# COPT-Public/LoRADS

Hardware: AMD Instinct MI355X
Metric: ADMM iters/sec (+ inner CG-iters/sec), single-block n=20000 r=40 (higher is better)
Workload: dtype f64

## Files before the change

### include/lorads_hip.h

```cpp
#ifndef LORADS_HIP_H
#define LORADS_HIP_H

#include <stdint.h>

#ifdef __cplusplus
extern "C" {
#endif

typedef struct lorads_hip_ctx lorads_hip_ctx;

typedef struct {
    int32_t n;
    int32_t rank;
    int32_t nrow;
    const int32_t *row_idx;
    const int32_t *a_ptr;
    const int32_t *a_row;
    const int32_t *a_col;
    const double *a_val;
    int32_t c_nnz;
    const int32_t *c_row;
    const int32_t *c_col;
    const double *c_val;
    int32_t is_lp;
// ... 19 lines not shown
void lorads_hip_destroy(lorads_hip_ctx *ctx);
const char *lorads_hip_last_error(void);

int lorads_hip_init_constr(lorads_hip_ctx *ctx, int32_t pair);
int lorads_hip_alm_cal_grad(lorads_hip_ctx *ctx, double rho, double *lag_norm_sq);
int lorads_hip_lbfgs_direction(lorads_hip_ctx *ctx, int32_t inner_iter);
int lorads_hip_alm_q12p12(lorads_hip_ctx *ctx, double p12[2]);
int lorads_hip_alm_linesearch_coeffs(lorads_hip_ctx *ctx, double rho, double p1, double p2, double coef[4]);
int lorads_hip_set_y_as_neg_grad(lorads_hip_ctx *ctx);
int lorads_hip_alm_update_var(lorads_hip_ctx *ctx, double tau);
int lorads_hip_set_lbfgs_his_two(lorads_hip_ctx *ctx, double tau);
int lorads_hip_update_dimacs(lorads_hip_ctx *ctx, int32_t pair, double *err1);
int lorads_hip_cal_obj(lorads_hip_ctx *ctx, int32_t pair, double *pobj);
int lorads_hip_alm_front(lorads_hip_ctx *ctx, double rho, int32_t inner, double out[6]);
int lorads_hip_alm_step(lorads_hip_ctx *ctx, double rho, double tau, int32_t next_inner, double out[8]);
int lorads_hip_admm_update_var(lorads_hip_ctx *ctx, double rho, double cg_tol, int32_t cg_max_iter,
                               int32_t *cg_iters);
int lorads_hip_admm_step(lorads_hip_ctx *ctx, double rho, double cg_tol, int32_t cg_max_iter, double out[4]);
int lorads_hip_update_dual_var(lorads_hip_ctx *ctx, double rho);
int lorads_hip_cal_dual_obj(lorads_hip_ctx *ctx, double *dobj);

int lorads_hip_dual_infeasibility(lorads_hip_ctx *ctx, double tol, int32_t ncv, int32_t max_restarts, double *sum_neg,
                                  double *lam_min, int32_t *matvecs);

#define LORADS_HIP_CERT_N 10
int lorads_hip_certificate(lorads_hip_ctx *ctx, int32_t src, double tol, int32_t ncv, int32_t max_restarts,
                           double out[LORADS_HIP_CERT_N], double *lam_min, double *residual, double *lambda);
int lorads_hip_get_slack(lorads_hip_ctx *ctx, int32_t blk, int64_t *nnz, int32_t *row, int32_t *col, double *val);

int lorads_hip_round_pm1(lorads_hip_ctx *ctx, int32_t src, int32_t trials, uint64_t seed, int32_t max_rounds, double *obj,
                         double *obj0, int32_t *best, int32_t *best0, int8_t *sign, int32_t *rounds, double *hyperplanes);

int lorads_hip_round_kcut(lorads_hip_ctx *ctx, int32_t src, int32_t parts, int32_t trials, uint64_t seed, int32_t max_rounds,
                          double *obj, double *obj0, int32_t *best, int32_t *best0, uint8_t *label, int32_t *rounds, double *vectors,
                          double *t, double *lp_upper);

int lorads_hip_round_stable(lorads_hip_ctx *ctx, int32_t src, int32_t trials, uint64_t seed, int32_t max_rounds, double *obj,
                            double *obj0, int32_t *best, int32_t *best0, uint8_t *member, int32_t *sizes, int32_t *rounds,
                            double *scores, double *T);

int lorads_hip_round_bisect(lorads_hip_ctx *ctx, int32_t src, int32_t trials, uint64_t seed, int32_t max_rounds, double *obj,
                            double *obj0, int32_t *best, int32_t *best0, int8_t *sign, int32_t *imbalance, int32_t *rounds,
                            double *hyperplanes, double *t, int32_t *diff);

int lorads_hip_spectrum(lorads_hip_ctx *ctx, int32_t src, double *eig, double *q, int32_t *sweeps);
int lorads_hip_compress_rank(lorads_hip_ctx *ctx, int32_t src, const int32_t *new_rank, double *eig);

#define LORADS_HIP_PRIMAL_CHUNK 262144
#define LORADS_HIP_PRIMAL_EPW 128
int lorads_hip_primal_entries(lorads_hip_ctx *ctx, int32_t src, int32_t blk, int64_t count, const int32_t *row, const int32_t *col,
                              double *val, const double *ref, double stats[4]);
int lorads_hip_primal_apply(lorads_hip_ctx *ctx, int32_t src, int32_t blk, int32_t ncols, const double *B, double *Y, double *T);

int lorads_hip_triangle_cuts(lorads_hip_ctx *ctx, int32_t src, int32_t blk, double min_violation, int32_t max_cuts, int64_t *count,
                             int32_t *p, int32_t *q, int32_t *s, int8_t *cls, double *viol, int32_t *kept, int32_t *passes);

int lorads_hip_entry_bounds(lorads_hip_ctx *ctx, int32_t src, int32_t blk, double lower, double upper, double min_violation,
                            int32_t max_cuts, int64_t *count, int32_t *p, int32_t *q, int8_t *cls, double *viol, int32_t *kept,
                            int32_t *passes);

int lorads_hip_primal_topk(lorads_hip_ctx *ctx, int32_t src, int32_t blk, int32_t nq, const int32_t *row, int32_t col_lo, int32_t col_hi,
                           int32_t k, int32_t smallest, int32_t include_diag, const int64_t *skip_ptr, const int32_t *skip_col,
                           int32_t *idx, double *val, int32_t *found);

int lorads_hip_alm_to_admm(lorads_hip_ctx *ctx);
int lorads_hip_average_uv_to_v(lorads_hip_ctx *ctx);
int lorads_hip_scale_obj(lorads_hip_ctx *ctx, double s);
int lorads_hip_resize_rank(lorads_hip_ctx *ctx, const int32_t *new_rank);
int lorads_hip_set_mat(lorads_hip_ctx *ctx, int32_t which, int32_t blk, const double *colmajor);
int lorads_hip_get_mat(lorads_hip_ctx *ctx, int32_t which, int32_t blk, double *colmajor);
int lorads_hip_set_vec(lorads_hip_ctx *ctx, int32_t which, const double *v);
int lorads_hip_get_vec(lorads_hip_ctx *ctx, int32_t which, double *v);
int lorads_hip_set_allreduce(lorads_hip_ctx *ctx, lorads_hip_allreduce_fn fn, void *user);
void *lorads_hip_stream(lorads_hip_ctx *ctx);
int lorads_hip_set_allreduce_stream_ordered(lorads_hip_ctx *ctx, int32_t on);
int lorads_hip_set_separable(lorads_hip_ctx *ctx, int32_t on);
typedef int (*lorads_hip_scalar_exchange_fn)(void *user, double *vals, int32_t n);
int lorads_hip_set_scalar_exchange(lorads_hip_ctx *ctx, lorads_hip_scalar_exchange_fn fn, void *user);
int lorads_hip_selfcheck_allreduce(lorads_hip_ctx *ctx);

int lorads_hip_sync(lorads_hip_ctx *ctx);
int lorads_hip_spec_front_stats(lorads_hip_ctx *ctx, int64_t out[4]);
int lorads_hip_handover_stats(lorads_hip_ctx *ctx, int64_t out[2]);
int lorads_hip_row_deal_stats(lorads_hip_ctx *ctx, int32_t block, int out[3]);
int lorads_hip_wt_stores(lorads_hip_ctx *ctx, int *mask);
int lorads_hip_front_chain(lorads_hip_ctx *ctx, int *mask, int *effective);
int lorads_hip_dense_plan(lorads_hip_ctx *ctx, int32_t block, int64_t out[16]);

#ifdef __cplusplus
}
#endif
#endif
```

### lorads_amd/csrc/hip/build.inc

```
struct HostPattern {
    std::vector<int> erow, ecol;
    std::vector<int> e_ptr, e_con;
    std::vector<double> e_val;
    std::vector<int> adj_ptr, adj_col, adj_e;
};
#include "presolve.inc"

void unique_positions(const std::vector<std::pair<int, int>> &pos, std::vector<std::pair<int, int>> &uniq,
                      std::vector<int> &index) {
    std::vector<int> order(pos.size());
    for (size_t i = 0; i < pos.size(); ++i) order[i] = (int)i;
    std::sort(order.begin(), order.end(), [&](int a, int b) {
        if (pos[a].second != pos[b].second) return pos[a].second < pos[b].second;
        if (pos[a].first != pos[b].first) return pos[a].first < pos[b].first;
        return a < b;
    });
    uniq.clear();
    index.assign(pos.size(), -1);
    for (size_t k = 0; k < order.size(); ++k) {
        int i = order[k];
        if (uniq.empty() || uniq.back() != pos[i]) uniq.push_back(pos[i]);
        index[i] = (int)uniq.size() - 1;
    }
}
// ... 333 lines not shown
    }
    tm.lap("operator kind (diag / single entry / colouring)");
    if (!diag && !B.dense_a && build_gram(M, B, hb, a_e, B.pa.ne)) return 1;
    tm.lap("Gram");
    {
        int maxsz = 0;
        for (int i = 0; i < hb.nrow; ++i) maxsz = std::max(maxsz, hb.a_ptr[i + 1] - hb.a_ptr[i]);
        const char *force = getenv("LORADS_OP_CW");
        bool want = !diag && !B.entry_only && hb.nrow >= 256 && maxsz <= 512;
        if (force && !diag && !B.entry_only && hb.nrow > 0) want = force[0] == '1';
        if (B.dense_a) want = false;
        if (want) {
            std::vector<int> deg(B.n + 1, 0);
            for (int t = 0; t < B.na; ++t) {
                deg[hb.a_row[t] + 1]++;
                if (hb.a_row[t] != hb.a_col[t]) deg[hb.a_col[t] + 1]++;
            }
            std::vector<int> ptr(B.n + 1, 0);
            for (int i = 0; i < B.n; ++i) ptr[i + 1] = ptr[i] + deg[i + 1];
            std::vector<int> col(ptr[B.n]), con(ptr[B.n]), fill(ptr.begin(), ptr.end() - 1);
            std::vector<double> av(ptr[B.n]);
            for (int i = 0; i < hb.nrow; ++i)
                for (int t = hb.a_ptr[i]; t < hb.a_ptr[i + 1]; ++t) {
                    const int p = hb.a_row[t], q = hb.a_col[t];
                    col[fill[p]] = q; con[fill[p]] = i; av[fill[p]] = hb.a_val[t]; fill[p]++;
                    if (p != q) { col[fill[q]] = p; con[fill[q]] = i; av[fill[q]] = hb.a_val[t]; fill[q]++; }
                }
            for (int i = 0; i < B.n; ++i) {
                const int s0 = ptr[i], s1 = ptr[i + 1];
                std::vector<std::tuple<int, int, double>> tmp(s1 - s0);
                for (int k = s0; k < s1; ++k) tmp[k - s0] = std::make_tuple(col[k], con[k], av[k]);
                std::sort(tmp.begin(), tmp.end());
                for (int k = s0; k < s1; ++k) { col[k] = std::get<0>(tmp[k - s0]); con[k] = std::get<1>(tmp[k - s0]); av[k] = std::get<2>(tmp[k - s0]); }
            }
            std::vector<int> car(hb.a_row, hb.a_row + B.na), cac(hb.a_col, hb.a_col + B.na);
            std::vector<double> cav(hb.a_val, hb.a_val + B.na);
            if (maxsz <= 32 && (double)hb.nrow * maxsz <= 1.5 * (double)B.na && !getenv("LORADS_NO_ELL")) {
                B.ca_ell = maxsz;
                car.assign((size_t)hb.nrow * maxsz, 0); cac.assign((size_t)hb.nrow * maxsz, 0); cav.assign((size_t)hb.nrow * maxsz, 0.0);
                for (int i = 0; i < hb.nrow; ++i)
                    for (int t = hb.a_ptr[i]; t < hb.a_ptr[i + 1]; ++t) {
                        const size_t w = (size_t)i * maxsz + (size_t)(t - hb.a_ptr[i]);
                        car[w] = hb.a_row[t]; cac[w] = hb.a_col[t]; cav[w] = hb.a_val[t];
                    }
            }
            if (!getenv("LORADS_NO_SLOT_ELL")) {
                long over8 = 0;
                for (int i = 0; i < B.n; ++i) over8 += (ptr[i + 1] - ptr[i]) > 8;
                const int ew = (double)over8 <= 0.005 * (double)B.n ? 8 : 16;
                std::vector<int> ecol((size_t)B.n * ew), econ((size_t)B.n * ew, 0);
                std::vector<double> eav((size_t)B.n * ew, 0.0);
                for (int i = 0; i < B.n; ++i)
                    for (int s = 0; s < ew; ++s) {
                        const int k = ptr[i] + s;
                        const size_t w = (size_t)i * ew + s;
                        if (k < ptr[i + 1]) { ecol[w] = col[k]; econ[w] = con[k]; eav[w] = av[k]; }
                        else ecol[w] = i;
                    }
                if (M.upload(&B.cell_col, ecol) || M.upload(&B.cell_con, econ) || M.upload(&B.cell_a, eav)) return 1;
                B.cell_w = ew;
            }
            if (B.cell_w && !B.dense_c && !getenv("LORADS_NO_FRONT_CW_DATA")) {
                std::vector<std::pair<int, int>> posC(B.nc), uniqC;
                for (int t = 0; t < B.nc; ++t) posC[t] = {hb.c_row[t], hb.c_col[t]};
                std::vector<int> cidx;
                unique_positions(posC, uniqC, cidx);
                std::vector<double> cval(uniqC.size(), 0.0);
                for (int t = 0; t < B.nc; ++t) cval[cidx[t]] += hb.c_val[t];
                HostPattern hpC;
                build_adjacency(B.n, uniqC, hpC);
                std::vector<double> fval(hpC.adj_e.size());
                for (size_t k = 0; k < hpC.adj_e.size(); ++k) fval[k] = cval[hpC.adj_e[k]];
                std::vector<int> ccount(hb.nrow, 0);
                for (int k = 0; k < ptr[B.n]; ++k) ccount[con[k]]++;
                int csw = 1;
                for (int i = 0; i < hb.nrow; ++i) csw = std::max(csw, ccount[i]);
                if ((double)hb.nrow * csw > 4.0 * (double)ptr[B.n] + 1024.0) csw = 0;
                if (csw > 0) {
                    std::vector<int> dstc(ptr[B.n]), fillc(hb.nrow, 0), dste((size_t)B.n * B.cell_w, 0);
                    for (int k = 0; k < ptr[B.n]; ++k) dstc[k] = con[k] * csw + fillc[con[k]]++;
                    for (int i = 0; i < B.n; ++i)
                        for (int sl = 0; sl < B.cell_w && ptr[i] + sl < ptr[i + 1]; ++sl) dste[(size_t)i * B.cell_w + sl] = dstc[ptr[i] + sl];
                    if (M.upload(&B.fc_ptr, hpC.adj_ptr) || M.upload(&B.fc_col, hpC.adj_col) || M.upload(&B.fc_val, fval) ||
                        M.upload(&B.cadj_dst, dstc) || M.upload(&B.cell_dst, dste) || M.alloc(&B.w_contrib, (size_t)hb.nrow * csw))
                        return 1;
                    HC(hipMemset(B.w_contrib, 0, sizeof(double) * std::max<size_t>((size_t)hb.nrow * csw, 1)));
                    B.cs_w = csw;
                    B.fc_nslot = (int)fval.size();
                    B.front_cw = true;
                }
            }
            if (M.upload(&B.ca_row, car) || M.upload(&B.ca_col, cac) || M.upload(&B.ca_val, cav) ||
                M.upload(&B.cadj_ptr, ptr) || M.upload(&B.cadj_col, col) || M.upload(&B.cadj_con, con) || M.upload(&B.cadj_a, av) ||
                M.alloc(&B.w_uv, (size_t)B.nrow) || M.alloc(&B.w_op, (size_t)B.nrow) || M.alloc(&B.pu.S2, (size_t)2 * B.pu.ne))
                return 1;
            B.cadj_ptr_host_n = ptr[B.n];
            B.use_cw = true;
        }
    }
    tm.lap("constraint-wise operator lists");
    if (hb.is_lp) {
        for (int t = 0; t < B.na; ++t)
            if (hb.a_row[t] != hb.a_col[t]) return fail_msg("LP block: off-diagonal entry");
        for (int t = 0; t < B.nc; ++t)
            if (hb.c_row[t] != hb.c_col[t]) return fail_msg("LP block: off-diagonal objective entry");
        const int n = B.n;
        std::vector<int> ptr(n + 1, 0), grow(B.na), fill(n, 0);
        std::vector<double> av(B.na), nrm(n, 0.0), cobj(n, 0.0);
        for (int t = 0; t < B.na; ++t) ptr[hb.a_row[t] + 1]++;
        for (int j = 0; j < n; ++j) ptr[j + 1] += ptr[j];
        for (int i = 0; i < hb.nrow; ++i)
            for (int t = hb.a_ptr[i]; t < hb.a_ptr[i + 1]; ++t) {
                const int col = hb.a_row[t], w = ptr[col] + fill[col]++;
                grow[w] = hb.row_idx[i];
                av[w] = hb.a_val[t];
            }
        for (int j = 0; j < n; ++j) {
            double nn = 0.0;
            for (int t = ptr[j]; t < ptr[j + 1]; ++t) nn += av[t] * av[t];
            const double nr = std::sqrt(nn);
            nrm[j] = nr * nr;
        }
        for (int t = 0; t < B.nc; ++t) cobj[hb.c_row[t]] += hb.c_val[t];
        std::vector<int> row_lvl((size_t)std::max(c->m, 1), 0), lvl(n, 0);
        int nlev = 0;
        for (int j = 0; j < n; ++j) {
            int l = 0;
            for (int t = ptr[j]; t < ptr[j + 1]; ++t) l = std::max(l, row_lvl[grow[t]]);
            lvl[j] = l;
            for (int t = ptr[j]; t < ptr[j + 1]; ++t) row_lvl[grow[t]] = l + 1;
            nlev = std::max(nlev, l + 1);
        }
        std::vector<int> lptr(nlev + 1, 0), lcols(n);
        for (int j = 0; j < n; ++j) lptr[lvl[j] + 1]++;
        for (int l = 0; l < nlev; ++l) lptr[l + 1] += lptr[l];
        std::vector<int> lf(lptr.begin(), lptr.end() - 1);
        for (int j = 0; j < n; ++j) lcols[lf[lvl[j]]++] = j;
        if (M.upload(&B.lp_ptr, ptr) || M.upload(&B.lp_grow, grow) || M.upload(&B.lp_a, av) || M.upload(&B.lp_nrm2sq, nrm) ||
            M.upload(&B.lp_cobj, cobj) || M.upload(&B.lp_lvl_ptr, lptr) || M.upload(&B.lp_lvl_cols, lcols) ||
            M.alloc(&B.lp_cv, (size_t)B.na))
            return 1;
        HC(hipMemset(B.lp_cv, 0, sizeof(double) * (size_t)std::max(B.na, 1)));
        B.is_lp = true;
        B.lp_nlev = nlev;
    }
    return 0;
}

void block_bytes(Block &B) {
    double F = 8.0 * B.n * B.r;
    B.bytes_mv = 4 * F + 32.0 * B.na + 16.0 * B.nrow;
    B.bytes_cg = B.bytes_mv + 9 * F;
}

inline int pad_rows(int n) { return (n + 31) & ~31; }

void common_rank(lorads_hip_ctx *c) {
    if (!c->merged_ok || c->nb < 2 || !env_on("LORADS_COMMON_RANK")) return;
    int rmax = 0;
    for (auto &B : c->blk) rmax = std::max(rmax, B.r);
    for (auto &B : c->blk) B.r = rmax;
}

int alloc_factors(lorads_hip_ctx *c) {
    c->all_elem = 0;
    for (auto &B : c->blk) {
        B.off = c->all_elem;
// ... 164 lines not shown
```

### lorads_amd/csrc/hip/dev.inc

```
int lorads_hip_ubench(lorads_hip_ctx *c, int32_t which, int32_t reps, double *ms) {
    spec_touch(c);
    if (c->nb < 1) return fail_msg("ubench: no cone");
    Block &B = c->blk[0];
    if (which >= 100) {
        if (!B.entry_only) return fail_msg("ubench: variants >= 100 need a single-entry cone");
        hipEvent_t e0, e1;
        HC(hipEventCreate(&e0)); HC(hipEventCreate(&e1));
        if (which != 100 && which != 120 && which != 121) return fail_msg("ubench: unknown variant");
        const Shape shp = shape_for(B.r);
        for (int it = -3; it < reps; ++it) {
            if (it == 0) HC(hipEventRecord(e0, c->stream));
            if (which == 100)
                op_entry(c, B, c->V + B.off, OP_CG, c->U + B.off, nullptr, c->cQ + B.off, part_slot(c, 0), NOGUARD);
            else
                SHAPE_DISPATCH(shp, LAUNCH((k_gather_probe<LG_, V2_, NS_>), nblocks_for((size_t)B.n, TPB / shp.lg), B.n, 16, B.pa.adj_col,
                                           B.na, c->V + B.off, which == 121 ? c->U + B.off : (const double *)nullptr, B.r,
                                           c->cQ + B.off));
        }
        HC(hipEventRecord(e1, c->stream));
        HC(hipEventSynchronize(e1));
        float f = 0;
        HC(hipEventElapsedTime(&f, e0, e1));
        *ms = f;
        hipEventDestroy(e0); hipEventDestroy(e1);
        return 0;
    }
    if (B.r != 40 || !B.use_cw || !B.cell_w || !B.pu.S2) return fail_msg("ubench: needs a k_cw cone of rank 40");
    const double *U = c->U + B.off, *V = c->V + B.off;
    double *Q = c->cQ + B.off, *r = c->cr + B.off, *p = c->cp + B.off, *rhs = c->rhs + B.off;
    const size_t len = (size_t)B.n * B.r;
    hipLaunchKernelGGL(k_fill, dim3(64), dim3(TPB), 0, c->stream, (size_t)NSLOT * c->maxpart, 1.0, c->part);
    HC(hipMemsetAsync(c->st, 0, sizeof(CGState) * 2, c->stream));
    hipEvent_t e0, e1;
    HC(hipEventCreate(&e0)); HC(hipEventCreate(&e1));
    const int grow = nblocks_for((size_t)B.n, TPB / 8), gcw = nblocks_for((size_t)B.nrow, TPB / 64);
    const RowDeal rd = row_deal_of(c, B);
    for (int it = -3; it < reps; ++it) {
        if (it == 0) HC(hipEventRecord(e0, c->stream));
        switch (which) {
        case 0: LAUNCH((k_cw<8, true, 3>), gcw, B.nrow, B.a_ptr, B.ca_row, B.ca_val, B.ca_col, U, V, B.r, 1.0, B.w_op, (double *)nullptr,
                       (int)CV_SET, B.row_idx, (double *)nullptr, NOGUARD, B.ca_ell, InitArgs{}, ResArgs{}); break;
        case 1: LAUNCH((k_cw<4, true, 5, true>), gcw, B.nrow, B.a_ptr, B.ca_row, B.ca_val, B.ca_col, U, V, B.r, 1.0, B.w_op,
                       (double *)nullptr, (int)CV_SET, B.row_idx, (double *)nullptr, NOGUARD, B.ca_ell, InitArgs{}, ResArgs{}); break;
        case 2:
            if (B.cell_w == 8) LAUNCH((k_spmm_ell<8, true, 3, 8>), rd.grid, B.n, rd.rpw, B.cadj_ptr, B.cadj_col, B.cadj_con, B.cadj_a, B.cell_col,
                                      B.cell_con, B.cell_a, (const double *)B.w_op, V, B.r, (int)OP_CG, U, (const double *)nullptr, Q,
                                      part_slot(c, 0), NOGUARD);
            else LAUNCH((k_spmm_ell<8, true, 3, 16>), rd.grid, B.n, rd.rpw, B.cadj_ptr, B.cadj_col, B.cadj_con, B.cadj_a, B.cell_col, B.cell_con,
                        B.cell_a, (const double *)B.w_op, V, B.r, (int)OP_CG, U, (const double *)nullptr, Q, part_slot(c, 0), NOGUARD);
            break;
        case 30: case 31: case 33: case 34: {
            if (!B.front_cw) return fail_msg("ubench: cone without the one-kernel front's data");
            FrontCwArgs A{};
            A.fc_ptr = B.fc_ptr; A.fc_col = B.fc_col; A.fc_val = B.fc_val; A.sl_ptr = B.cadj_ptr; A.sl_col = B.cadj_col; A.sl_con = B.cadj_con;
            A.sl_a = B.cadj_a; A.ell_col = B.cell_col; A.ell_con = B.cell_con; A.ell_a = B.cell_a; A.ell_dst = B.cell_dst; A.sl_dst = B.cadj_dst;
            A.csum = c->csum; A.b = c->b; A.lambda = c->lambda; A.cv = B.cv; A.w_uv = B.w_op;
            A.row_idx = B.row_idx_identity ? nullptr : B.row_idx; A.rho = 1.0; A.wmode = W_ADMM;
            A.contrib = (which == 30 || which == 33) ? B.w_contrib : (double *)nullptr;
            A.wt = c->opt_wt_stores;
            const size_t lds = sizeof(double2) * 32 * 4 * 3 * 8;
#define UB_FRONT(EWV, FCV) LAUNCH_LDS((k_front_cw<3, EWV, 4, false, FCV>), rd.grid, lds, B.n, rd.rpw, A, V, B.r, U, r, rhs, part_slot(c, 0), part_slot(c, 1), NOGUARD, Deferred{})
            if (which < 33) { if (B.cell_w == 8) UB_FRONT(8, 0); else UB_FRONT(16, 0); }
            else { if (B.cell_w == 8) UB_FRONT(8, FC_ALL); else UB_FRONT(16, FC_ALL); }
#undef UB_FRONT
        } break;
        case 32: LAUNCH(k_wsum, nblocks_for((size_t)B.nrow, TPB / 8), B.nrow, B.cs_w, (const double *)B.w_contrib, B.w_op, NOGUARD, InitArgs{}, 0, DS(0.0),
                        c->m, (const double *)c->b, (const double *)c->csum, c->lambda); break;
        case 3: LAUNCH((k_spmm<8, true, 3, true>), grow, B.n, B.cadj_ptr, B.cadj_col, B.cadj_con, (const double *)B.w_op, V, B.r,
                       (int)OP_CG, U, (const double *)nullptr, 0.0, Q, part_slot(c, 0), NOGUARD, (const double *)nullptr, B.cadj_a); break;
        case 4: LAUNCH((k_spmm2<8, true, 3, true>), grow, B.n, B.pu.adj_ptr, B.pu.adj_col, B.pu.adj_dyn, B.pu.adj_sval, B.pu.S, (const double *)B.pu.S2, V,
                       B.r, 0, U, (const double *)nullptr, 1.0, r, rhs, part_slot(c, 0), part_slot(c, 1), NOGUARD,
                       (const double *)nullptr); break;
        case 5: LAUNCH((k_spmm2<8, true, 3, false>), grow, B.n, B.pu.adj_ptr, B.pu.adj_col, B.pu.adj_dyn, B.pu.adj_sval, B.pu.S, (const double *)nullptr, V,
                       B.r, (int)OP_RHS, (const double *)nullptr, (const double *)nullptr, 1.0, rhs, (double *)nullptr, part_slot(c, 1),
                       (double *)nullptr, NOGUARD, (const double *)nullptr); break;
        case 6: case 7: case 8: case 9: {
            const int gv = 2048 >> (which - 6);
            LAUNCH(k_cg_update<true>, gv, len, c->st, part_slot(c, 0), 625, Q, rhs, p, r, part_slot(c, 2), NOGUARD, (double *)nullptr,
                   (const double *)nullptr, 0, c->st_shadow);
        } break;
        case 20: case 21: case 22: case 23: case 24: {
            const bool shortk = which >= 23;
            const int ngroups = shortk ? B.n : 40000, per = shortk ? 16 : 64;
            const double *two = (which == 21 || which == 24) ? U : (const double *)nullptr;
            const int *idx = which == 22 ? (const int *)nullptr : B.cadj_col;
            const int nidx = which == 22 ? B.n : B.cadj_ptr_host_n;
            if (nidx <= 0) return fail_msg("ubench: empty index list");
            LAUNCH((k_gather_probe<8, true, 3>), nblocks_for((size_t)ngroups, TPB / 8), ngroups, per, idx, nidx, V, two, B.r, Q);
        } break;
        case 25: LAUNCH((k_gather_probe2<8, true, 3, 0>), grow, B.n, B.pu.adj_ptr, B.pu.adj_col, B.pu.adj_e, B.pu.S, V, B.r, Q); break;
        case 26: LAUNCH((k_gather_probe2<8, true, 3, 1>), grow, B.n, B.pu.adj_ptr, B.pu.adj_col, B.pu.adj_e, B.pu.S, V, B.r, Q); break;
        case 27: LAUNCH((k_gather_probe2<8, true, 3, 3>), grow, B.n, B.pu.adj_ptr, B.pu.adj_col, B.pu.adj_e, B.pu.S, V, B.r, Q); break;
        case 28: LAUNCH((k_gather_probe2<8, true, 3, 7>), grow, B.n, B.pu.adj_ptr, B.pu.adj_col, B.pu.adj_e, B.pu.S, V, B.r, Q); break;
        case 10: case 13: case 14:
            LAUNCH((k_obj<8, true, 3>), std::min(nblocks_for((size_t)B.nc, TPB / 8), which == 10 ? 1024 : which == 13 ? 2048 : 4096), B.nc,
                   B.c_row, B.c_col, B.c_val, U, U, B.r, part_slot(c, 4), NOGUARD); break;
        case 11: LAUNCH(k_sval, std::max(1, nblocks_for((size_t)B.pu.ne, TPB)), B.pu.ne, B.pu.e_ptr, B.pu.e_con, B.pu.e_val, B.pu.cbase,
                        (int)W_COMPACT, WArgs{B.w_op, nullptr, nullptr, nullptr, nullptr, nullptr, 1.0}, B.pu.S, NOGUARD,
                        (CGState *)nullptr, 0, (const double *)B.w_op, B.pu.S2); break;
        default: return fail_msg("ubench: unknown variant");
        }
    }
    HC(hipEventRecord(e1, c->stream));
    HC(hipEventSynchronize(e1));
    float f = 0;
    HC(hipEventElapsedTime(&f, e0, e1));
    *ms = f;
    hipEventDestroy(e0); hipEventDestroy(e1);
    invalidate_t(c);
    return 0;
}
```

### lorads_amd/csrc/hip/kernels.inc

```
template <int LG, bool V2, int NS>
struct Slice {
    static constexpr int W = V2 ? 2 : 1;
    __device__ static __forceinline__ void load(const double *__restrict__ row, int r, int lane, double (&v)[NS][W]) {
#pragma unroll
        for (int c = 0; c < NS; ++c) {
            const int j = (lane + c * LG) * W;
            const bool ok = j < r;
            const int jc = ok ? j : 0;
            if (V2) {
                const double2 t = *(const double2 *)(row + jc);
                v[c][0] = ok ? t.x : 0.0;
                v[c][W - 1] = ok ? t.y : 0.0;
            } else {
                const double t = row[jc];
                v[c][0] = ok ? t : 0.0;
            }
        }
    }
    __device__ static __forceinline__ void load_raw(const double *__restrict__ row, int r, int lane, double (&v)[NS][W]) {
        static_assert(V2, "the 16-byte form only");
#pragma unroll
        for (int c = 0; c < NS; ++c) {
            const int j = (lane + c * LG) * W;
            const double2 t = *(const double2 *)(row + (j < r ? j : 0));
// ... 62 lines not shown
    double *part_v, *part_d;
};
template <int LG, bool V2, int NS, bool ONE = false>
__global__ __launch_bounds__(TPB) void k_cw(int nrow, const int *__restrict__ a_ptr, const int *__restrict__ a_p,
                                            const double *__restrict__ a_val, const int *__restrict__ a_q,
                                            const double *__restrict__ X,
                                            const double *__restrict__ Y, int r, double scale, double *__restrict__ w_out,
                                            double *__restrict__ cv, int mode, const int *__restrict__ row_idx,
                                            double *__restrict__ vec, Guard g, int ell_w, InitArgs ia, ResArgs ra,
                                            Deferred d = Deferred{}) {
    __shared__ double sh[8];
    DefPriv dv{};
    if (d.st) dv = deferred_private(d);
    const Gate gt = gate_load(ia.st ? Guard{nullptr, g.need} : g);
    double iv[2] = {0.0, 0.0};
    const bool ia_small = ia.st && ia.nrr <= 4 * TPB && ia.nb <= 4 * TPB;
    double ipr[2][4] = {{0.0, 0.0, 0.0, 0.0}, {0.0, 0.0, 0.0, 0.0}};
    if (ia_small) {
#pragma unroll
        for (int k = 0; k < 4; ++k) {
            const int j = threadIdx.x + k * TPB;
            ipr[0][k] = ia.part_rr[j < ia.nrr ? j : 0];
            ipr[1][k] = ia.part_b[j < ia.nb ? j : 0];
        }
    } else if (ia.st) init_private(ia, iv);
    constexpr int GR = 64 / LG;
    const int i = (blockIdx.x * TPB + threadIdx.x) >> 6, lane64 = threadIdx.x & 63;
    const int grp = lane64 / LG, lane = lane64 % LG;
    const bool act = i < nrow;
    const int ic = act ? i : 0;
    int gi_pre = 0;
    double b_pre = 0.0, l_pre = 0.0;
    if (ra.b) { gi_pre = row_idx[ic]; b_pre = ra.b[gi_pre]; l_pre = ra.lambda[gi_pre]; }
    const int t0 = ell_w ? ic * ell_w : a_ptr[ic], t1 = !act ? t0 : ell_w ? t0 + ell_w : a_ptr[ic + 1];
    double acc = 0.0;
    if (ONE) {
        for (int t = t0 + grp; t < t1; t += GR) {
            const int p0 = a_p[t], q0 = a_q[t];
            const double c0 = a_val[t];
            acc += c0 * pair_dot<LG, V2, NS>(X, Y, p0, q0, r, lane);
        }
    } else
    for (int t = t0 + grp; t < t1; t += 2 * GR) {
        const int tb = t + GR < t1 ? t + GR : t;
        const int p0 = a_p[t], q0 = a_q[t], p1 = a_p[tb], q1 = a_q[tb];
        const double c0 = a_val[t], c1 = t + GR < t1 ? a_val[tb] : 0.0;
        const double d0 = pair_dot<LG, V2, NS>(X, Y, p0, q0, r, lane);
        const double d1 = pair_dot<LG, V2, NS>(X, Y, p1, q1, r, lane);
        acc += c0 * d0;
        acc += c1 * d1;
    }
    const double s = wave_sum(acc);
    if (ia_small) {
#pragma unroll
        for (int k = 0; k < 4; ++k) {
            const int j = threadIdx.x + k * TPB;
            iv[0] += j < ia.nrr ? ipr[0][k] : 0.0;
            iv[1] += j < ia.nb ? ipr[1][k] : 0.0;
        }
    }
    const bool live = ia.st ? finish_init(ia, !(g.need && gt.vn == 0), iv, sh) == 0
                            : d.st ? !blocked_after(g, d, finish_deferred(d, dv, sh).done) : GATE_OPEN;
    if (live && act && lane64 == 0) {
        if (w_out) w_out[i] = s;
        if (vec) {
            const int gi = ra.b ? gi_pre : row_idx[i];
            if (mode == CV_SET) vec[gi] = s * scale;
            else if (mode == CV_ADD) vec[gi] += s * scale;
            else vec[gi] += s - cv[i];
        }
        if (cv) cv[i] = s;
    }
    if (ra.b) {
        double vd[2] = {0.0, 0.0};
        if (act && lane64 == 0) {
            const double bi = b_pre, t = bi - s * scale;
            vd[0] = t * t;
            vd[1] = bi * l_pre;
        }
        block_sum_n<2>(vd, sh);
        if (live && threadIdx.x == 0) { ra.part_v[blockIdx.x] = vd[0]; ra.part_d[blockIdx.x] = vd[1]; }
    }
}

template <int NS4, int NS>
__global__ __launch_bounds__(TPB) void k_eval_cw_obj(int nrow, int ell_w, const int *__restrict__ a_p, const double *__restrict__ a_val,
                                                     const int *__restrict__ a_q, const double *__restrict__ R, int r,
                                                     double *__restrict__ cv, const int *__restrict__ row_idx, double *__restrict__ vec,
                                                     ResArgs ra, int g_cw, int ne, const int *__restrict__ erow,
                                                     const int *__restrict__ ecol, const double *__restrict__ cval,
                                                     double *__restrict__ part_obj, Guard g, Deferred d) {
    __shared__ double sh[8];
    const Gate gt = gate_load(g);
    DefPriv dv{};
    if (d.st) dv = deferred_private(d);
    if ((int)blockIdx.x < g_cw) {
        constexpr int LG = 4, GR = 16;
        const int i = (blockIdx.x * TPB + threadIdx.x) >> 6, lane64 = threadIdx.x & 63;
        const int grp = lane64 / LG, lane = lane64 % LG;
        const bool act = i < nrow;
        const int ic = act ? i : 0;
        const int gi = row_idx[ic];
        const double bi = ra.b[gi], li = ra.lambda[gi];
        const int t0 = ic * ell_w, t1 = act ? t0 + ell_w : t0;
        double acc = 0.0;
        for (int t = t0 + grp; t < t1; t += GR) {
            const int p0 = a_p[t], q0 = a_q[t];
            const double c0 = a_val[t];
            acc += c0 * pair_dot<LG, true, NS4>(R, R, p0, q0, r, lane);
        }
        const double s = wave_sum(acc);
        const bool live = d.st ? !blocked_after(g, d, finish_deferred(d, dv, sh).done) : GATE_OPEN;
        if (live && act && lane64 == 0) { vec[gi] = s * 1.0; cv[i] = s; }
        double vd[2] = {0.0, 0.0};
        if (act && lane64 == 0) {
            const double t = bi - s * 1.0;
            vd[0] = t * t;
            vd[1] = bi * li;
        }
        block_sum_n<2>(vd, sh);
        if (live && threadIdx.x == 0) { ra.part_v[blockIdx.x] = vd[0]; ra.part_d[blockIdx.x] = vd[1]; }
        return;
    }
    constexpr int LG = 8, per = TPB / LG;
    const int bid = blockIdx.x - g_cw, nblk = gridDim.x - g_cw;
    const int lane = threadIdx.x % LG;
    double sacc = 0.0;
    for (int e = bid * per + threadIdx.x / LG; e < ne; e += nblk * per)
        sacc += pair_dot<LG, true, NS>(R, R, erow[e], ecol[e], r, lane) * cval[e];
    const bool live = d.st ? !blocked_after(g, d, finish_deferred(d, dv, sh).done) : GATE_OPEN;
    const double t = block_sum(sacc, sh);
    if (live && threadIdx.x == 0) part_obj[bid] = t;
}

__global__ void k_fill(size_t len, double v, double *__restrict__ y) {
    for (size_t i = (size_t)blockIdx.x * blockDim.x + threadIdx.x; i < len; i += (size_t)gridDim.x * blockDim.x) y[i] = v;
}

template <int LG, bool V2, int NS>
__device__ __forceinline__ void pair_dot_rd(const double *__restrict__ R, const double *__restrict__ D, int p, int q, int r,
                                            int lane, double &t1, double &t2) {
    constexpr int W = V2 ? 2 : 1;
    double rp[NS][W], rq[NS][W], dp[NS][W], dq[NS][W];
    Slice<LG, V2, NS>::load(R + (size_t)p * r, r, lane, rp);
    Slice<LG, V2, NS>::load(D + (size_t)q * r, r, lane, dq);
    Slice<LG, V2, NS>::load(R + (size_t)q * r, r, lane, rq);
    Slice<LG, V2, NS>::load(D + (size_t)p * r, r, lane, dp);
    double a1 = 0.0, a2 = 0.0, b1 = 0.0, b2 = 0.0;
#pragma unroll
    for (int c = 0; c < NS; ++c)
#pragma unroll
        for (int w = 0; w < W; ++w) {
            a1 += rp[c][w] * dq[c][w]; a2 += rq[c][w] * dp[c][w];
            b1 += dp[c][w] * dq[c][w]; b2 += dq[c][w] * dp[c][w];
        }
    t1 = p == q ? a1 : a1 + a2;
    t2 = p == q ? b1 : b1 + b2;
}
template <int LG, bool V2, int NS>
__global__ __launch_bounds__(TPB) void k_pairdots_rd(int ne, const int *__restrict__ erow, const int *__restrict__ ecol,
                                                     const double *__restrict__ R, const double *__restrict__ D, int r,
                                                     double *__restrict__ T1, double *__restrict__ T2) {
    const int e = (blockIdx.x * TPB + threadIdx.x) / LG, lane = threadIdx.x % LG;
    const bool act = e < ne;
    const int p = act ? erow[e] : 0, q = act ? ecol[e] : 0;
    double t1, t2;
// ... 356 lines not shown
                for (int u = 0; u < CH; ++u) {
                    const double a1 = __shfl(s1, u0 + u, 8);
                    const double a2 = FRONT ? __shfl(s2, u0 + u, 8) : 0.0;
#pragma unroll
                    for (int c = 0; c < NS; ++c)
#pragma unroll
                        for (int w = 0; w < W; ++w) {
                            acc[c][w] += a1 * v[u][c][w];
                            if (FRONT) acc2[c][w] += a2 * v[u][c][w];
                        }
                }
            }
        }
    }
    const bool live_ = (FRONT && d.st) ? !blocked_after(g, d, finish_deferred(d, dv, sh).done) : GATE_OPEN;
    double dd = 0.0;
    if (FRONT && gd) {
#pragma unroll
        for (int c = 0; c < NS; ++c)
#pragma unroll
            for (int w = 0; w < W; ++w) dd += rh[c][w] * xi[c][w];
        dd = group_sum<LG>(dd);
        if (uv_out && act && lane == 0 && live_) uv_out[rowc] = dd;
        dd *= gd[rowc];
    }
    double local = 0.0, local_b = 0.0;
#pragma unroll
    for (int c = 0; c < NS; ++c) {
        const int j0 = (lane + c * LG) * W;
        double v[W], vb[W];
#pragma unroll
        for (int w = 0; w < W; ++w) {
            const double a = acc[c][w];
            if (FRONT) {
                vb[w] = xi[c][w] - a / rho; local_b += fabs(vb[w]);
                const double opx = gd ? rh[c][w] + dd * xi[c][w] : rh[c][w] + acc2[c][w];
                v[w] = vb[w] - opx; local += v[w] * v[w];
            } else if (mode == OP_CG) { v[w] = xi[c][w] + a; local += xi[c][w] * v[w]; }
            else if (mode == OP_RES) { v[w] = rh[c][w] - (xi[c][w] + a); local += v[w] * v[w]; }
            else if (mode == OP_RHS) { v[w] = xi[c][w] - a / rho; local += fabs(v[w]); }
            else { v[w] = 2.0 * a; local += v[w] * v[w]; }
        }
        if (live_ && act && j0 < r) {
            if (V2) *(double2 *)(out + base + j0) = make_double2(v[0], v[W - 1]);
            else out[base + j0] = v[0];
            if (FRONT) {
                if (V2) *(double2 *)(rhs_out + base + j0) = make_double2(vb[0], vb[W - 1]);
                else rhs_out[base + j0] = vb[0];
            }
        }
    }
    if (FRONT) {
        double two[2] = {act ? local : 0.0, act ? local_b : 0.0};
        block_sum_n<2>(two, sh);
        if (live_ && threadIdx.x == 0) { part[blockIdx.x] = two[0]; part_b[blockIdx.x] = two[1]; }
    } else {
        const double t = block_sum(act ? local : 0.0, sh);
        if (live_ && threadIdx.x == 0) part[blockIdx.x] = t;
    }
}

struct Cg0Args {
    const CGState *st;
    const double *part_ww;
    int nww;
    double *x, *r;
    int store_r;
    double *w_acc;
    const double *w_p;
    int nw;
    CGState *shadow;
    const double *avg_other;
    double *avg_out;
    int wt;
};
struct CgElem { double x, r; };
__device__ __forceinline__ CgElem cg_elem(double alpha, double p, double q, double x, double r) {
    return CgElem{x + alpha * p, r - alpha * q};
}
__device__ __forceinline__ double cg_avg(double other, double x) { return (other + x) / 2; }
__device__ __forceinline__ double cg_wacc(double wa, double alpha, double wp) { return wa + alpha * wp; }
__device__ __forceinline__ double cg0_alpha(double rr, double ww) { return rr / (rr + ww); }

template <int LG, bool V2, int NS, int EW, bool CG0 = false>
__global__ __launch_bounds__(TPB) void k_spmm_ell(int n, int rpw, const int *__restrict__ adj_ptr, const int *__restrict__ adj_col,
                                                  const int *__restrict__ adj_con, const double *__restrict__ adj_a,
                                                  const int *__restrict__ ell_col, const int *__restrict__ ell_con,
                                                  const double *__restrict__ ell_a, const double *__restrict__ wgt,
                                                  const double *__restrict__ X, int r, int mode,
                                                  const double *xin, const double *__restrict__ rhs,
                                                  double *__restrict__ out, double *__restrict__ part, Guard g,
                                                  Cg0Args u = Cg0Args{}) {
    __shared__ double sh[4];
    const Gate gt = gate_load(g);
    double rr = 0.0, ww = 0.0, wa0 = 0.0, wp0 = 0.0;
    const int gid = blockIdx.x * TPB + threadIdx.x;
    if (CG0) {
        rr = u.st->rr;
        ww = private_partials(u.part_ww, u.nww);
        if (u.w_acc) { const int iw = gid < u.nw ? gid : 0; wa0 = u.w_acc[iw]; wp0 = u.w_p[iw]; }
    }
    constexpr int W = V2 ? 2 : 1;
    constexpr int NH = EW / 8;
    constexpr int CH = NS <= 5 ? 4 : 2;
    const int grp = threadIdx.x / LG, row = blockIdx.x * rpw + grp, lane = threadIdx.x % LG;
    const bool act = grp < rpw && row < n;
    const int rowc = act ? row : 0;
    const size_t base = (size_t)rowc * r;
    const size_t eb = (size_t)rowc * EW + (lane & 7);
    int qc[NH], kc[NH];
    double ac[NH];
#pragma unroll
    for (int h = 0; h < NH; ++h) { qc[h] = ell_col[eb + 8 * h]; kc[h] = ell_con[eb + 8 * h]; ac[h] = ell_a[eb + 8 * h]; }
    const int t0 = adj_ptr[rowc], t1r = adj_ptr[rowc + 1];
    const int t1 = act ? t1r : t0;
    double xi[NS][W], rh[NS][W], acc[NS][W];
    Slice<LG, V2, NS>::load(xin + base, r, lane, xi);
    Slice<LG, V2, NS>::load((CG0 ? (const double *)u.x : mode == OP_RES ? rhs : xin) + base, r, lane, rh);
#pragma unroll
    for (int c = 0; c < NS; ++c)
#pragma unroll
        for (int w = 0; w < W; ++w) acc[c][w] = 0.0;
    double wv[NH];
#pragma unroll
    for (int h = 0; h < NH; ++h) wv[h] = wgt[kc[h]];
    const int cnt = act ? t1 - t0 : 0;
#pragma unroll
    for (int h = 0; h < NH; ++h) {
        if (h == 0 || cnt > 8 * h) {
#pragma unroll
            for (int u0 = 0; u0 < 8; u0 += CH) {
                if (u0 > 0 && cnt <= 8 * h + u0) continue;
                double v[CH][NS][W];
#pragma unroll
                for (int u = 0; u < CH; ++u) {
                    const int q = __shfl(qc[h], u0 + u, 8);
                    Slice<LG, V2, NS>::load(X + (size_t)q * r, r, lane, v[u]);
                }
                const double sch = (lane & 7) + 8 * h < cnt ? ac[h] * wv[h] : 0.0;
#pragma unroll
                for (int u = 0; u < CH; ++u) {
                    const double su = __shfl(sch, u0 + u, 8);
#pragma unroll
                    for (int c = 0; c < NS; ++c)
#pragma unroll
                        for (int w = 0; w < W; ++w) acc[c][w] += su * v[u][c][w];
                }
            }
        }
    }
    constexpr int TU = CG0 ? 2 : 4;
    for (int t = t0 + EW; t < t1; t += TU) {
        int q[TU], e[TU];
        double aa[TU];
#pragma unroll
        for (int u = 0; u < TU; ++u) {
            const int tt = t + u < t1 ? t + u : t1 - 1;
            q[u] = adj_col[tt];
            e[u] = adj_con[tt];
            aa[u] = adj_a[tt];
        }
        double s4[TU], v[TU][NS][W];
#pragma unroll
        for (int u = 0; u < TU; ++u) {
            s4[u] = aa[u] * wgt[e[u]];
            Slice<LG, V2, NS>::load(X + (size_t)q[u] * r, r, lane, v[u]);
        }
#pragma unroll
        for (int u = 0; u < TU; ++u) {
            const double su = t + u < t1 ? s4[u] : 0.0;
#pragma unroll
            for (int c = 0; c < NS; ++c)
#pragma unroll
                for (int w = 0; w < W; ++w) acc[c][w] += su * v[u][c][w];
        }
    }
    if (CG0) {
        const double alpha = cg0_alpha(rr, block_sum(ww, sh));
        const bool open = GATE_OPEN;
        const bool avg_only = !open && gt.vs != 0 && !(g.need && gt.vn == 0);
        if (open && blockIdx.x == 0 && threadIdx.x == 0 && u.shadow) *u.shadow = *u.st;
        if (open && u.w_acc && gid < u.nw) {
            u.w_acc[gid] = cg_wacc(wa0, alpha, wp0);
            for (int i = gid + gridDim.x * TPB; i < u.nw; i += gridDim.x * TPB) u.w_acc[i] = cg_wacc(u.w_acc[i], alpha, u.w_p[i]);
        }
        double local = 0.0;
#pragma unroll
        for (int c = 0; c < NS; ++c) {
            const int j0 = (lane + c * LG) * W;
            double xo[W], ro[W];
#pragma unroll
            for (int w = 0; w < W; ++w) {
                const CgElem e = cg_elem(alpha, xi[c][w], xi[c][w] + acc[c][w], rh[c][w], xi[c][w]);
                xo[w] = e.x; ro[w] = e.r;
                local += e.r * e.r;
            }
            if (act && j0 < r) {
                if (open) {
                    if (V2) store16(u.x, base + j0, xo[0], xo[W - 1], u.wt & WT_CG0);
                    else store8(u.x, base + j0, xo[0], u.wt & WT_CG0);
                    if (u.store_r) {
                        if (V2) store16(u.r, base + j0, ro[0], ro[W - 1], u.wt & WT_CG0);
                        else store8(u.r, base + j0, ro[0], u.wt & WT_CG0);
                    }
                }
                if (u.avg_out && (open || avg_only)) {
                    double ao[W];
#pragma unroll
                    for (int w = 0; w < W; ++w) ao[w] = open ? xo[w] : rh[c][w];
                    if (V2) {
                        const double2 o = *(const double2 *)(u.avg_other + base + j0);
                        store16(u.avg_out, base + j0, cg_avg(o.x, ao[0]), cg_avg(o.y, ao[W - 1]), u.wt & WT_AVG);
                    } else {
                        store8(u.avg_out, base + j0, cg_avg(u.avg_other[base + j0], ao[0]), u.wt & WT_AVG);
                    }
                }
            }
        }
        const double t = block_sum(act ? local : 0.0, sh);
        if (open && threadIdx.x == 0) part[blockIdx.x] = t;
        return;
    }
    double local = 0.0;
#pragma unroll
    for (int c = 0; c < NS; ++c) {
        const int j0 = (lane + c * LG) * W;
        double v[W];
#pragma unroll
        for (int w = 0; w < W; ++w) {
            const double a = acc[c][w];
            if (mode == OP_CG) { v[w] = xi[c][w] + a; local += xi[c][w] * v[w]; }
            else { v[w] = rh[c][w] - (xi[c][w] + a); local += v[w] * v[w]; }
        }
        if (GATE_OPEN && act && j0 < r) {
            if (V2) store16(out, base + j0, v[0], v[W - 1], u.wt & WT_OUT);
            else store8(out, base + j0, v[0], u.wt & WT_OUT);
        }
    }
    const double t = block_sum(act ? local : 0.0, sh);
    if (GATE_OPEN && threadIdx.x == 0) part[blockIdx.x] = t;
}

struct FrontCwArgs {
    const int *fc_ptr, *fc_col;
    const double *fc_val;
    const int *sl_ptr;
    const int *sl_col, *sl_con;
    const double *sl_a;
    const int *ell_col, *ell_con;
    const double *ell_a;
    const int *ell_dst, *sl_dst;
    const double *csum, *b, *lambda, *cv, *w_uv;
    const int *row_idx;
    DS rho, rho_dual;
    int dual_on;
    int wmode;
    double *contrib;
    CGState *reset;
    int nreset;
    int wt;
};
__device__ __forceinline__ void front_cw_weights(const FrontCwArgs &A, double rho, double rho_dual, int i, double a, double &c1, double &c2) {
    const int g = A.row_idx ? A.row_idx[i] : i;
    const double cs0 = A.csum[g], bb = A.b[g], lam0 = A.lambda[g], cvv = A.cv[i], wu = A.w_uv[i];
    double m1;
    if (A.wmode == W_ADMM_V) {
        const double cs = cs0 + (wu - cvv);
        m1 = ((cs - bb) - wu) * rho - lam0;
    } else {
        double lam = lam0;
        if (A.dual_on) { const double l = lam0 + rho_dual * bb; lam = l + (-rho_dual) * cs0; }
        m1 = ((cs0 - bb) - cvv) * rho - lam;
    }
    c1 = a * m1;
    c2 = a * wu;
}
struct EvalFinalArgs {
    const double *part_v, *part_d, *obj_part;
    int np, nobj;
    double *out;
    Guard g;
};
__device__ __forceinline__ void publish_final(EvalFinalArgs fa, const unsigned long long *src, int nwords, unsigned long long *dst,
                                              unsigned long long *flag, unsigned long long *seq_dev, double *sh) {
    const unsigned long long seq = *seq_dev + 1;
    constexpr int PW = 4;
    unsigned long long pre[PW];
#pragma unroll
    for (int k = 0; k < PW; ++k) {
        const int i = threadIdx.x + k * TPB;
        pre[k] = __builtin_nontemporal_load(src + (i < nwords ? i : 0));
    }
    const bool live = !blocked(fa.g);
    const double *const pp[3] = {fa.part_v, fa.part_d, fa.obj_part ? fa.obj_part : fa.part_v};
    const int nn[3] = {fa.np, fa.np, fa.obj_part ? fa.nobj : 0};
    double t3[3];
    private_partials_n<3>(pp, nn, t3);
    block_sum_n<3>(t3, sh);
    const double v = t3[0], d = t3[1], o = t3[2];
    if (live && threadIdx.x == 0) { fa.out[0] = v; fa.out[1] = d; if (fa.obj_part) fa.out[2] = o; }
    const bool own = (const double *)src == fa.out;
#pragma unroll
    for (int k = 0; k < PW; ++k) {
        const int i = threadIdx.x + k * TPB;
        if (i >= nwords) continue;
        unsigned long long w = pre[k];
        if (live && own) {
            if (i == 0) w = (unsigned long long)__double_as_longlong(v);
            else if (i == 1) w = (unsigned long long)__double_as_longlong(d);
            else if (i == 2 && fa.obj_part) w = (unsigned long long)__double_as_longlong(o);
        }
        dst[i] = w;
    }
    if (!own || nwords > PW * TPB) {
        __threadfence();
        __syncthreads();
        for (int i = threadIdx.x; i < nwords; i += TPB) dst[i] = __builtin_nontemporal_load(src + i);
    }
    __threadfence_system();
    __syncthreads();
    if (threadIdx.x == 0) {
        *seq_dev = seq;
        __atomic_store_n(flag, seq, __ATOMIC_RELEASE);
        __threadfence_system();
    }
}
struct HandoverArgs {
    EvalFinalArgs fa;
    const unsigned long long *src;
    unsigned long long *dst;
    int nwords;
    unsigned long long *flag, *seq_dev;
    int lead;
};
struct FrontCwHoArgs : FrontCwArgs { HandoverArgs ho; };
enum { FC_RAW = 1, FC_LATE = 2, FC_ALL = 3, FC_DEFAULT = FC_ALL };
template <int NB, class SL, bool RAW = false, int NS, int W>
__device__ __forceinline__ void front_gather(const double *__restrict__ X, int r, int lane, int q, int u0, double (&v)[NB][NS][W]) {
#pragma unroll
    for (int u = 0; u < NB; ++u) {
        if constexpr (RAW) SL::load_raw(X + (size_t)__shfl(q, u0 + u, 8) * r, r, lane, v[u]);
        else SL::load(X + (size_t)__shfl(q, u0 + u, 8) * r, r, lane, v[u]);
    }
}
template <int NB, int NS, int W>
__device__ __forceinline__ void front_fma2(double k1, double k2, int u0, const double (&v)[NB][NS][W], double (&acc)[NS][W], double (&acc2)[NS][W]) {
#pragma unroll
    for (int u = 0; u < NB; ++u) {
        const double s1 = __shfl(k1, u0 + u, 8), s2 = __shfl(k2, u0 + u, 8);
#pragma unroll
        for (int c = 0; c < NS; ++c)
#pragma unroll
            for (int w = 0; w < W; ++w) { acc[c][w] += s1 * v[u][c][w]; acc2[c][w] += s2 * v[u][c][w]; }
    }
}
template <int NB, int NS, int W>
__device__ __forceinline__ void front_dots(const double (&r0)[NS][W], const double (&v)[NB][NS][W], int u0, int l8, double &mine) {
#pragma unroll
    for (int u = 0; u < NB; ++u) {
        double dsum = 0.0;
#pragma unroll
        for (int c = 0; c < NS; ++c)
#pragma unroll
            for (int w = 0; w < W; ++w) dsum += r0[c][w] * v[u][c][w];
        dsum = group_sum<8>(dsum);
        mine = l8 == u0 + u ? dsum : mine;
    }
}
template <int NS, int EW, int KC = 0, bool HO = false, int FC = 0>
__global__ __launch_bounds__(TPB) void k_front_cw(int n, int rpw, std::conditional_t<HO, FrontCwHoArgs, FrontCwArgs> A,
                                                  const double *__restrict__ X, int r,
                                                  const double *__restrict__ xin, double *__restrict__ out,
                                                  double *__restrict__ rhs_out, double *__restrict__ part,
                                                  double *__restrict__ part_b, Guard g, Deferred d) {
    constexpr int LG = 8, W = 2, NH = EW / 8;
    constexpr bool RAW = (FC & FC_RAW) != 0, LATE = (FC & FC_LATE) != 0;
    using SL = Slice<LG, true, NS>;
    __shared__ double sh[HO ? 12 : 8];
    extern __shared__ __attribute__((aligned(16))) double2 slotc[];
    unsigned wg = blockIdx.x;
    if constexpr (HO) {
        if (blockIdx.x < (unsigned)A.ho.lead) {
            if (blockIdx.x == 0) publish_final(A.ho.fa, A.ho.src, A.ho.nwords, A.ho.dst, A.ho.flag, A.ho.seq_dev, sh);
            return;
        }
        wg = blockIdx.x - A.ho.lead;
    }
    if (A.reset && wg == 0 && threadIdx.x < A.nreset) A.reset[threadIdx.x].done = 0;
    const Gate gt = gate_load(g);
    const double rho = dsv(A.rho), rho_dual = A.dual_on ? dsv(A.rho_dual) : 0.0;
    DefPriv dv{};
    if (d.st) dv = deferred_private(d);
    const int grp = threadIdx.x / LG, row = wg * rpw + grp, lane = threadIdx.x % LG, l8 = lane & 7;
    const bool act = grp < rpw && row < n;
    const int rowc = act ? row : 0;
    const size_t base = (size_t)rowc * r;
    const int c0 = A.fc_ptr[rowc], c1e = act ? A.fc_ptr[rowc + 1] : c0;
    const int a0 = A.sl_ptr[rowc], a1r = A.sl_ptr[rowc + 1];
    const int a1 = act ? a1r : a0;
    const int cnt = a1 - a0;
    const size_t eb = (size_t)rowc * EW + l8;
    int qc[NH], kc[NH], dc[NH];
    double ac[NH];
#pragma unroll
    for (int h = 0; h < NH; ++h) { qc[h] = A.ell_col[eb + 8 * h]; kc[h] = A.ell_con[eb + 8 * h]; ac[h] = A.ell_a[eb + 8 * h]; dc[h] = A.ell_dst[eb + 8 * h]; }
    int tn = c0 + l8, tc = tn < c1e ? tn : (c1e > 0 ? c1e - 1 : 0);
    int qn = A.fc_col[tc];
    double svn = A.fc_val[tc];
    double xi[NS][W], rh[NS][W];
    if constexpr (!LATE) {
        SL::load(X + base, r, lane, xi);
        SL::load(xin + base, r, lane, rh);
    }
    double k1[NH], k2[NH];
#pragma unroll
    for (int h = 0; h < NH; ++h) {
        front_cw_weights(A, rho, rho_dual, kc[h], ac[h], k1[h], k2[h]);
        const bool mine = l8 + 8 * h < cnt;
        k1[h] = mine ? k1[h] : 0.0;
        k2[h] = mine ? k2[h] : 0.0;
    }
    double acc[NS][W], acc2[NS][W];
#pragma unroll
    for (int c = 0; c < NS; ++c)
#pragma unroll
        for (int w = 0; w < W; ++w) { acc[c][w] = 0.0; acc2[c][w] = 0.0; }
    for (int t = c0; t < c1e; t += 8) {
        const int q = qn;
        const double sv = t + l8 < c1e ? svn : 0.0;
        tn = t + 8 + l8;
        tc = tn < c1e ? tn : c1e - 1;
        qn = A.fc_col[tc];
        svn = A.fc_val[tc];
#pragma unroll
        for (int u0 = 0; u0 < 8; u0 += 4) {
            if (u0 == 0 || t + u0 < c1e) {
                double v[4][NS][W];
                front_gather<4, SL, RAW>(X, r, lane, q, u0, v);
#pragma unroll
                for (int u = 0; u < 4; ++u) {
                    const double a1c = __shfl(sv, u0 + u, 8);
#pragma unroll
                    for (int c = 0; c < NS; ++c)
#pragma unroll
                        for (int w = 0; w < W; ++w) acc[c][w] += a1c * v[u][c][w];
                }
            }
        }
    }
    {
        double v[4][NS][W];
        front_gather<4, SL, RAW>(X, r, lane, qc[0], 0, v);
        if constexpr (LATE) {
            SL::load(X + base, r, lane, xi);
            SL::load(xin + base, r, lane, rh);
        }
        if constexpr (KC > 0) {
#pragma unroll
            for (int u = 0; u < 4; ++u)
#pragma unroll
                for (int c = 0; c < NS; ++c)
                    slotc[(((threadIdx.x >> 3) * KC + u) * NS + c) * 8 + l8] = make_double2(v[u][c][0], v[u][c][1]);
        }
        front_fma2<4>(k1[0], k2[0], 0, v, acc, acc2);
    }
    if (cnt > 4) {
        double v[4][NS][W];
        front_gather<4, SL, RAW>(X, r, lane, qc[0], 4, v);
        front_fma2<4>(k1[0], k2[0], 4, v, acc, acc2);
    }
#pragma unroll
    for (int h = 1; h < NH; ++h) {
        if (cnt > 8 * h) {
#pragma unroll
            for (int u0 = 0; u0 < 8; u0 += 4) {
                if (u0 > 0 && cnt <= 8 * h + u0) continue;
                double v[4][NS][W];
                front_gather<4, SL, RAW>(X, r, lane, qc[h], u0, v);
                front_fma2<4>(k1[h], k2[h], u0, v, acc, acc2);
            }
        }
    }
    for (int t = a0 + EW; t < a1; ++t) {
        double s1, s2, v[NS][W];
        front_cw_weights(A, rho, rho_dual, A.sl_con[t], A.sl_a[t], s1, s2);
        if constexpr (RAW) SL::load_raw(X + (size_t)A.sl_col[t] * r, r, lane, v);
        else SL::load(X + (size_t)A.sl_col[t] * r, r, lane, v);
#pragma unroll
        for (int c = 0; c < NS; ++c)
#pragma unroll
            for (int w = 0; w < W; ++w) { acc[c][w] += s1 * v[c][w]; acc2[c][w] += s2 * v[c][w]; }
    }
    const bool live = d.st ? !blocked_after(g, d, finish_deferred(d, dv, sh).done) : GATE_OPEN;
    double r0[NS][W];
    double local = 0.0, local_b = 0.0;
#pragma unroll
    for (int c = 0; c < NS; ++c) {
        const int j0 = (lane + c * LG) * W;
        double vb[W];
#pragma unroll
        for (int w = 0; w < W; ++w) {
            vb[w] = xi[c][w] - acc[c][w] / rho;
            r0[c][w] = vb[w] - (rh[c][w] + acc2[c][w]);
            if constexpr (RAW) {
                vb[w] = j0 < r ? vb[w] : 0.0;
                r0[c][w] = j0 < r ? r0[c][w] : 0.0;
            }
            local_b += fabs(vb[w]);
            local += r0[c][w] * r0[c][w];
        }
        if (live && act && j0 < r) {
            store16(out, base + j0, r0[c][0], r0[c][1], A.wt & WT_R0);
            store16(rhs_out, base + j0, vb[0], vb[1], A.wt & WT_RHS);
        }
    }
    const int cnt2 = A.contrib ? cnt : 0;
    const int a1b = A.contrib ? a1 : a0;
    if (cnt2 > 0) {
        double mine = 0.0;
        if constexpr (KC > 0) {
            double v[4][NS][W];
#pragma unroll
            for (int u = 0; u < 4; ++u)
#pragma unroll
                for (int c = 0; c < NS; ++c) {
                    const double2 t = slotc[(((threadIdx.x >> 3) * KC + u) * NS + c) * 8 + l8];
                    v[u][c][0] = t.x; v[u][c][1] = t.y;
                }
            front_dots<4>(r0, v, 0, l8, mine);
            if (cnt2 > 4) {
                front_gather<4, SL, RAW>(X, r, lane, qc[0], 4, v);
                front_dots<4>(r0, v, 4, l8, mine);
            }
        } else {
#pragma unroll
            for (int u0 = 0; u0 < 8; u0 += 4) {
                if (u0 > 0 && cnt2 <= u0) continue;
                double v[4][NS][W];
                front_gather<4, SL, RAW>(X, r, lane, qc[0], u0, v);
                front_dots<4>(r0, v, u0, l8, mine);
            }
        }
        if (live && l8 < cnt2) store8(A.contrib, (size_t)dc[0], ac[0] * mine, A.wt & WT_CONTRIB);
    }
#pragma unroll
    for (int h = 1; h < NH; ++h) {
        if (cnt2 > 8 * h) {
            double mine = 0.0;
#pragma unroll
            for (int u0 = 0; u0 < 8; u0 += 4) {
                if (u0 > 0 && cnt2 <= 8 * h + u0) continue;
                double v[4][NS][W];
                front_gather<4, SL, RAW>(X, r, lane, qc[h], u0, v);
                front_dots<4>(r0, v, u0, l8, mine);
            }
            if (live && l8 + 8 * h < cnt2) store8(A.contrib, (size_t)dc[h], ac[h] * mine, A.wt & WT_CONTRIB);
        }
    }
    for (int t = a0 + EW; t < a1b; ++t) {
        double v[NS][W], dsum = 0.0;
        SL::load(X + (size_t)A.sl_col[t] * r, r, lane, v);
#pragma unroll
        for (int c = 0; c < NS; ++c)
#pragma unroll
            for (int w = 0; w < W; ++w) dsum += r0[c][w] * v[c][w];
        dsum = group_sum<LG>(dsum);
        if (live && l8 == 0) store8(A.contrib, (size_t)A.sl_dst[t], A.sl_a[t] * dsum, A.wt & WT_CONTRIB);
    }
// ... 1618 lines not shown
```

### lorads_amd/csrc/hip/lorads_hip.hip

```cpp
#include <hip/hip_runtime.h>

#include <fcntl.h>
#include <sys/file.h>
#include <unistd.h>

#include <algorithm>
#include <chrono>
#include <cmath>
#include <cstdint>
#include <cstdio>
#include <cstring>
#include <map>
#include <string>
#include <atomic>
#include <mutex>
#include <thread>
#include <tuple>
#include <type_traits>
#include <utility>
#include <vector>

#include "lorads_hip.h"
#include "lorads_hip_dev.h"

// ... 241 lines not shown
#include "dev_kernels.inc"
#endif

#include "dev_pool.inc"

struct Pattern {
    int ne = 0;
    int nslot = 0;
    int n_owned = 0;
    int *erow = nullptr, *ecol = nullptr;
    int *e_ptr = nullptr, *e_con = nullptr;
    int *e_con_own = nullptr;
    double *e_val = nullptr;
    int *adj_ptr = nullptr, *adj_col = nullptr, *adj_e = nullptr;
    int *adj_dyn = nullptr;
    double *adj_sval = nullptr;
    double *S = nullptr;
    double *S2 = nullptr;
    double *cbase = nullptr;
};

struct Block {
    int n = 0, r = 0, nrow = 0, na = 0, nc = 0;
    int rl = 0;
    size_t off = 0;
    int *row_idx = nullptr;
    bool row_idx_identity = false;
    bool sv_direct = false;
    int *sv_ptr = nullptr, *sv_e = nullptr;
    double *sv_a = nullptr;
    int *a_ptr = nullptr, *a_e = nullptr;
    double *a_val = nullptr;
    Pattern pa, pu;
    bool has_gram = false;
    int *g_ptr = nullptr, *g_col = nullptr;
    double *g_val = nullptr;
    double *T = nullptr;
    double *cv = nullptr;
    double *wtmp = nullptr;
    int *c_row = nullptr, *c_col = nullptr;
    double *c_val = nullptr;
    bool dense_c = false;
    int npad = 0;
    double *Cfull = nullptr;
    double *Wd = nullptr;
    double *Wpart = nullptr;
    int ksplit_b = 0;
    bool dense_a = false;
    int nd = 0;
    int *d_con = nullptr;
    std::vector<int> d_con_h;
    double *Adense = nullptr;
    double *Sfull = nullptr;
    double *d_mu = nullptr;
    double *Wj = nullptr;
    double *Wc = nullptr;
    const double *wj_for = nullptr;
    bool t_uv_valid = false;
    double *T2 = nullptr;
    bool diag_only = false;
    double *gdiag = nullptr;
    int *diag_row = nullptr;
    int rc_w = 0;
    int *rc_con = nullptr;
    double *diag_a = nullptr;
    bool use_cw = false;
    int *cadj_ptr = nullptr, *cadj_col = nullptr, *cadj_con = nullptr;
    int *ca_row = nullptr, *ca_col = nullptr;
    double *ca_val = nullptr;
    int ca_ell = 0;
    double *cadj_a = nullptr;
    int cadj_ptr_host_n = 0;
    int cell_w = 0;
    int *cell_col = nullptr, *cell_con = nullptr;
    double *cell_a = nullptr;
    double *w_uv = nullptr, *w_op = nullptr;
    bool front_cw = false;
    int *fc_ptr = nullptr, *fc_col = nullptr;
    double *fc_val = nullptr;
    int fc_nslot = 0;
    int cs_w = 0;
    int *cell_dst = nullptr, *cadj_dst = nullptr;
    double *w_contrib = nullptr;
    bool w0_ready = false;
    bool is_lp = false;
    int lp_nlev = 0;
    int *lp_lvl_ptr = nullptr, *lp_lvl_cols = nullptr, *lp_ptr = nullptr, *lp_grow = nullptr;
    double *lp_a = nullptr, *lp_nrm2sq = nullptr, *lp_cobj = nullptr, *lp_cv = nullptr;
    bool entry_only = false;
    double *gentry = nullptr;
    int *bip_rows[2] = {nullptr, nullptr};
    int bip_n[2] = {0, 0};
    double *bip_we = nullptr;
    int cg_iter_last = 0;
    int spec[2] = {1, 1};
    int spec_hist[2][8] = {{1, 1, 1, 1, 1, 1, 1, 1}, {1, 1, 1, 1, 1, 1, 1, 1}};
    int spec_pos = 0;
    double bytes_mv = 0, bytes_cg = 0;
};

struct Ring {
    double *s = nullptr, *y = nullptr;
};
struct GraphCache;
struct PersistPlan;
struct LTeamPlan;

class Pending {
public:
    struct Dir { int kind = 0; CGState *st = nullptr; double *r = nullptr, *p = nullptr; size_t len = 0; int gv = 0;
                 const double *rs_part = nullptr; int rs_np = 0; Guard g{}; bool seg = false; int half = 0;
                 const double *chk_part = nullptr; double chk_tol = 0; int chk_maxit = 0, chk_k = 0;
                 const double *rs_seg = nullptr; };
    struct SegChk { bool on = false; int half = 0, k = 0; const double *part = nullptr; double tol = 0; int maxit = 0;
                    bool ride_res = false; };
    struct SegInit { bool on = false; int half = 0; double tol = 0; Guard front{}; const double *part_rr = nullptr, *part_b = nullptr; };
    bool must_flush() const { return init.st || chk.st || dir.kind || dual || dual_virtual || sep || seginit.on; }
    bool at_rest_for_replay() const { return !init.st && !chk.st && !dir.kind && !segchk.on && !dual_virtual; }
    void restore(Pending from) { from.dual_rho = dual_rho; from.sep = sep; from.sep_with_obj = sep_with_obj; from.sep_ex = sep_ex; *this = from; }
    void post_init(lorads_hip_ctx *c, CGState *st, const double *part_rr, int nrr, const double *part_b, int nb, double tol, Guard front);
    void post_check(lorads_hip_ctx *c, CGState *st, const double *part, int np, double tol, int maxit, Guard g);
    void post_dir(const Dir &d) { dir = d; }
    void post_segchk(const SegChk &t) { segchk = t; }
    void post_seginit(const SegInit &t) { seginit = t; }
    void post_dual(double rho) { dual = true; dual_rho = rho; }
    void post_sep(int with_obj, const SepExtra &ex) { sep = true; sep_with_obj = with_obj; sep_ex = ex; }
    InitArgs take_init_on(const Guard &g) { return (init.st && !chk.st && g.skip == &init.st->done && g.need == init_g.need) ? std::exchange(init, InitArgs{}) : InitArgs{}; }
    Deferred take_check_on(const Guard &g) { return take_check(chk.st && !init.st && g.skip == &chk.st->done && g.need == chk_g.need); }
    Deferred take_check_behind(const Guard &g) { return take_check(chk.st && !init.st && !dir.kind && !g.skip && g.need == &chk.st->done); }
    Deferred take_check_of(const CGState *st) { return take_check(chk.st == st && !init.st); }
    DirArgs take_on_op_diag(lorads_hip_ctx *c, int mode, const double *xin, const Guard &g, int rows);
    const double *take_segchk_part(int half, int k) {
        return segchk_is(half, k) ? std::exchange(segchk, SegChk{}).part : nullptr;
    }
    bool segchk_rides_res(int half, int k) { return segchk_is(half, k) && (segchk.ride_res = true); }
    bool take_sep(int max_extra, int *with_obj, SepExtra *ex) {
        if (!sep || sep_ex.n > max_extra) return false;
        sep = false; *with_obj = sep_with_obj; *ex = sep_ex;
        return true;
    }
    bool dual_rides(const Guard &front, bool lockstep = false) const {
        return dual && !front.need && !front.skip && !init.st && !chk.st && !dir.kind && (!lockstep || (!segchk.on && !dual_virtual));
    }
    bool dual_owed_unused() const { return dual && !dual_virtual; }
    bool dual_owed() const { return dual || dual_virtual; }
    bool dual_owed_at(double rho) const { return dual && memcmp(&dual_rho, &rho, sizeof(double)) == 0; }
    double dual_rho_value() const { return dual_rho; }
    double take_dual() { dual = false; return dual_rho; }
    double use_dual() { dual = false; dual_virtual = true; return dual_rho; }
    bool take_dual_used(double *rho) { const bool was = set_dual_used(false); if (was) *rho = dual_rho; return was; }
    bool set_dual_used(bool on) { const bool was = dual_virtual; dual_virtual = on; return was; }
    bool sep_waits() const { return sep; }
    void flush(lorads_hip_ctx *c);
    void flush_segchk(lorads_hip_ctx *c);
private:
    Deferred take_check(bool may) { return may ? std::exchange(chk, Deferred{}) : Deferred{}; }
    bool segchk_is(int half, int k) const { return segchk.on && segchk.half == half && segchk.k == k; }
    InitArgs init{}; Guard init_g{};
    Deferred chk{}; Guard chk_g{};
    Dir dir;
    SegChk segchk;
    SegInit seginit;
    bool dual = false, dual_virtual = false;
    double dual_rho = 0.0;
    bool sep = false; int sep_with_obj = 0; SepExtra sep_ex{};
};
// ... 179 lines not shown
    double *R = nullptr, *U = nullptr, *V = nullptr, *G = nullptr;
    double *cr = nullptr, *cp = nullptr, *cQ = nullptr, *rhs = nullptr;
    double *Dtmp = nullptr;
    double *cstage = nullptr;
    bool stage_clean = false;
    int ar_fast_all = -1;
    bool opt_ar_fast = true;
    double *b = nullptr, *lambda = nullptr, *csum = nullptr, *q12 = nullptr;
    double *part = nullptr;
    int maxpart = MINPART;
    int ls_np = 0;
    char *ctrl = nullptr, *h_ctrl = nullptr;
    char *h_ctrl_dev = nullptr;
    unsigned long long *h_flag = nullptr, *h_flag_dev = nullptr, pub_seq = 0;
    unsigned long long *seq_dev = nullptr;
    double *par = nullptr;
    double par_h[4] = {0, 0, 0, 0};
    int par_valid = 0;
    bool par_mode = false;
    const char *launch_err = nullptr;
    bool par_changed_last = false;
    double par_req[3] = {0, 0, 0};
    bool par_req_valid = false;
    bool opt_graph = true;
    bool opt_graph_batched = false;
    bool opt_graph_forced = false;
    GraphCache *graphs = nullptr;
    PersistPlan *persist = nullptr;
    bool opt_persist = true;
    int shared_gpu_fd = -1;
    bool opt_persist_carry = true;
    bool opt_persist_l2 = true;
    int opt_persist_rows = 0;
    bool opt_persist_linear = false;
    bool persist_stamps = false;
    long long n_persist = 0;
    long long n_launch = 0;
    LTeamPlan *lteam = nullptr;
    bool opt_lbfgs_team = true;
    bool opt_alm_sval_direct = true;
    bool opt_alm_fold_cv = true;
    bool opt_alm_fused_tail = true;
    bool use_publish = true;
    Pending pend;
    double *lambda_alt = nullptr;
    bool virt_refresh = false;
    bool opt_entry_bip = true;
    bool opt_fuse_dir = true;
    bool opt_cw_quad = true;
    bool opt_fuse_eval = true;
    bool opt_dense_rem = true;
    bool opt_pad_rank = true;
    bool opt_dev_presolve = true;
    bool opt_presolve_check = false;
    size_t dev_presolve_min = (size_t)1 << 15;
    long long n_dev_patterns = 0, n_checked_patterns = 0;
    bool opt_bisect_lds = true;
    bool opt_dense_cache = true;
    bool opt_front_diag = true;
    bool opt_eval_diag = true;
    bool opt_fold_avg = true;
    bool opt_tile_update = true;
    bool avg_folded = false;
    bool opt_front_lds = true;
    bool opt_front_cw = true;
    bool opt_fuse_cg0 = true;
    int opt_row_deal = -1, row_deal_cus = 0;
    int opt_wt_stores = WT_DEFAULT;
    int opt_front_chain = FC_DEFAULT;
    bool opt_spec_front = true;
    struct SpecFront {
        bool live = false;
        bool dual_seen = false;
        double rho = 0.0, rho_dual = 0.0;
        int wmode = 0;
        unsigned long long epoch = 0;
        CGState *reset = nullptr;
        int nreset = 0;
    } spec;
    unsigned long long spec_epoch = 0;
    long long n_spec_enq = 0, n_spec_adopt = 0, n_spec_discard = 0, n_spec_blocked = 0;
    bool opt_handover_on_front = true;
    long long n_handover_front = 0, n_handover_alone = 0;
    bool opt_exact_refresh = false, opt_split_front = false;
    bool final_pending = false;
    EvalFinalArgs final_args;
    double *scal = nullptr;
    CGState *st = nullptr;
    CGState *st_shadow = nullptr;
    bool opt_lazy_scalars = true;
    bool opt_seg_carry_init = true;
    lorads_hip_scalar_exchange_fn sx = nullptr;
    void *sx_user = nullptr;
    bool sx_pending = false;
    int sx_with_obj = 0;
    long long n_sx = 0;
    bool opt_seg_virt = true;
    bool opt_seg_carry_dual = true;
    bool opt_seg_carry_restart = true;
    double *seg_rr_alt = nullptr;
    int *seg_tile_info = nullptr;
    bool opt_seg_carry = true;
    int *seg_tile_cone = nullptr;
    CGState *h_st = nullptr;
    double *h_scal = nullptr;
    std::vector<Ring> ring;
    double *ring_ab = nullptr;
    int head = 0;
    lorads_hip_allreduce_fn ar = nullptr;
    void *ar_user = nullptr;
    bool ar_stream_ordered = false;
    bool sep = false;
    double *sepbuf = nullptr;
    SepExtra sep_extra{};
    double *gram = nullptr;
    bool opt_gram = true;
    bool opt_gram_single = false;
    int prof = 0, prof_every = 8;
    int prof_target = 0;
    long n_front = 0;
    long n_sweeps = 0;
    long n_matvec = 0, n_cg_it = 0, n_solves = 0, n_samp = 0, n_samp_spmm = 0, n_resume = 0;
    double ms_samp = 0, ms_samp_spmm = 0;
    std::vector<float> samp_ms;
    std::vector<std::pair<hipEvent_t, hipEvent_t>> timed_mv, timed_sp;
    std::vector<hipEvent_t> ev_pool;
    size_t ev_next = 0;
};

namespace {

inline DS ds_rho(const lorads_hip_ctx *c, double v) { return c->par_mode ? DS(c->par + 0, v) : DS(v); }
inline DS ds_tol(const lorads_hip_ctx *c, double v) { return c->par_mode ? DS(c->par + 1, v) : DS(v); }
inline DS ds_rho_dual(const lorads_hip_ctx *c, double v) { return c->par_mode ? DS(c->par + 2, v) : DS(v); }
inline DS ds_maxit(const lorads_hip_ctx *c, int v) { return c->par_mode ? DS(c->par + 3, (double)v) : DS((double)v); }
inline int nblocks_for(size_t items, int per_block) { return (int)((items + per_block - 1) / per_block); }
struct RowDeal { int rpw, grid; };
inline RowDeal row_deal(size_t n, int ncu) {
    const int g0 = nblocks_for(n, 32);
    if (ncu <= 0 || g0 <= ncu) return RowDeal{32, g0};
    const size_t k = ((size_t)g0 + ncu - 1) / ncu;
    const int rpw = (int)std::min<size_t>(32, (n + k * ncu - 1) / (k * ncu));
    return RowDeal{rpw, nblocks_for(n, rpw)};
}
inline int grid_lbfgs(size_t len);
inline int grid1d(size_t len) {
    size_t g = (len + TPB - 1) / TPB;
    return (int)std::min<size_t>(std::max<size_t>(g, 1), 2048);
}
inline int grid_lbfgs(size_t len) {
    return std::min(grid1d(len), 512);
}
inline bool use_v2(int r) { return (r % 2) == 0 && r <= 128; }
inline int lg_for(int r) { return use_v2(r) ? 8 : (r <= 64 ? 8 : (r <= 256 ? 32 : 64)); }
const Guard NOGUARD{nullptr, nullptr};

double *part_slot(lorads_hip_ctx *c, int k) { return c->part + (size_t)k * c->maxpart; }
inline bool shard_vec(const lorads_hip_ctx *c) { return c->ar && !c->sep; }
inline int dev_rank(const lorads_hip_ctx *c, int r, bool is_lp) { return (c->opt_pad_rank && !is_lp && (r & 1) && r < 512) ? r + 1 : r; }

inline void spec_touch(lorads_hip_ctx *c) {
    if (!c) return;
    if (c->spec.live) { c->spec.live = false; ++c->n_spec_discard; }
    ++c->spec_epoch;
}
inline void persist_touch(lorads_hip_ctx *c);
#include "build.inc"
#include "sweep.inc"
#include "persist.inc"
#include "lbfgs_team.inc"

int ctx_init(lorads_hip_ctx *c, const lorads_hip_problem *prob) {
    c->m = prob->m; c->nb = prob->nblocks; c->L = std::max(prob->lbfgs_len, 1); c->b_nrm1 = prob->b_nrm1;
    HC(hipStreamCreateWithFlags(&c->stream, hipStreamNonBlocking));
    {
        size_t rows_max = 0, rows_all = 0;
        for (int k = 0; k < c->nb; ++k) {
            const size_t nk = (size_t)std::max(prob->blocks[k].n, 0);
            rows_max = std::max(rows_max, nk);
            rows_all += (nk + 31) & ~(size_t)31;
        }
        const size_t need = (std::max(rows_max, rows_all) + 3) / 4 + 1;
        if (need > ((size_t)1 << 27)) return fail_msg("cone dimension beyond 2^29 rows");
        c->maxpart = (int)std::max<size_t>((size_t)MINPART, (need + 255) & ~(size_t)255);
    }
    c->opt_pad_rank = env_on("LORADS_PAD_ODD_RANK");
    c->opt_dev_presolve = env_on("LORADS_DEV_PRESOLVE");
    c->opt_presolve_check = env_set("LORADS_PRESOLVE_CHECK");
    if (getenv("LORADS_DEV_PRESOLVE_MIN")) c->dev_presolve_min = (size_t)std::max(0ll, atoll(getenv("LORADS_DEV_PRESOLVE_MIN")));
    c->blk.resize(c->nb);
    for (int k = 0; k < c->nb; ++k)
        if (build_block(c, c->blk[k], prob->blocks[k])) return 1;
    if (build_merged(c, prob)) return 1;
    common_rank(c);
    refresh_merged(c);
    if (getenv("LORADS_HIP_VERBOSE"))
        fprintf(stderr, "lorads_hip: %d cone(s), merged view %s\n", c->nb, c->has_merged ? "on" : (c->merged_ok ? "off (ranks differ)" : "not applicable"));
    if (alloc_factors(c)) return 1;
    std::vector<double> hb(prob->b, prob->b + c->m);
    DevPool &M = c->mem;
    if (M.upload(&c->b, hb) || M.alloc(&c->lambda, (size_t)c->m) || M.alloc(&c->lambda_alt, (size_t)c->m) || M.alloc(&c->csum, (size_t)c->m + 2) ||
        M.alloc(&c->cstage, (size_t)c->m + 2 + MINPART) || M.alloc(&c->gram, 128) ||
        M.alloc(&c->q12, (size_t)2 * c->m + 2) || M.alloc(&c->part, (size_t)NSLOT * c->maxpart) ||
        M.alloc(&c->ctrl, 64 * sizeof(double) + sizeof(CGState) * (size_t)std::max(2 * c->nb, 1)) ||
        M.alloc(&c->ring_ab, (size_t)2 * c->L) || M.alloc(&c->par, 8) || M.alloc(&c->seq_dev, 2))
        return 1;
    HC(hipMemset(c->par, 0, sizeof(double) * 8));
    HC(hipMemset(c->seq_dev, 0, sizeof(unsigned long long) * 2));
    c->opt_graph = env_on("LORADS_GRAPH");
    c->opt_graph_batched = getenv("LORADS_GRAPH") && getenv("LORADS_GRAPH")[0] == '2';
    c->opt_graph_forced = getenv("LORADS_GRAPH") && (getenv("LORADS_GRAPH")[0] == '1' || getenv("LORADS_GRAPH")[0] == '2');
    if (M.alloc_pinned(&c->h_ctrl, 64 * sizeof(double) + sizeof(CGState) * (size_t)std::max(2 * c->nb, 1), hipHostMallocMapped) ||
        M.alloc_pinned(&c->h_flag, 64 / sizeof(*c->h_flag), hipHostMallocMapped))
        return 1;
    *c->h_flag = 0;
    HC(hipHostGetDevicePointer((void **)&c->h_ctrl_dev, c->h_ctrl, 0));
    HC(hipHostGetDevicePointer((void **)&c->h_flag_dev, c->h_flag, 0));
    c->use_publish = !getenv("LORADS_NO_PUBLISH");
    c->opt_lazy_scalars = env_on("LORADS_LAZY_SCALARS");
    c->opt_ar_fast = !env_set("LORADS_AR_PLAIN");
    c->opt_gram = env_on("LORADS_LBFGS_GRAM");
    c->opt_gram_single = getenv("LORADS_LBFGS_GRAM") && getenv("LORADS_LBFGS_GRAM")[0] == '2';
    c->opt_fuse_dir = env_on("LORADS_FUSE_DIR");
    c->opt_entry_bip = env_on("LORADS_ENTRY_BIP");
    c->opt_seg_carry = env_on("LORADS_SEG_CARRY");
    c->opt_seg_carry_init = env_on("LORADS_SEG_CARRY_INIT");
    c->opt_seg_virt = env_on("LORADS_SEG_VIRT");
    c->opt_seg_carry_dual = env_on("LORADS_SEG_CARRY_DUAL");
    c->opt_seg_carry_restart = env_on("LORADS_SEG_CARRY_RESTART");
    c->opt_cw_quad = env_on("LORADS_CW_QUAD");
    c->opt_front_cw = env_on("LORADS_FRONT_CW");
    c->opt_fuse_cg0 = env_on("LORADS_FUSE_CG0");
    c->opt_front_lds = env_on("LORADS_FRONT_LDS");
    {
        const char *v = getenv("LORADS_ROW_DEAL");
        c->opt_row_deal = (!v || !v[0] || v[0] == 'a') ? -1 : std::max(0, std::min(32, atoi(v)));
        int dev = 0;
        HC(hipGetDevice(&dev));
        HC(hipDeviceGetAttribute(&c->row_deal_cus, hipDeviceAttributeMultiprocessorCount, dev));
        if (getenv("LORADS_ROW_DEAL_CUS")) c->row_deal_cus = std::max(1, atoi(getenv("LORADS_ROW_DEAL_CUS")));
    }
    if (getenv("LORADS_WT_STORES") && getenv("LORADS_WT_STORES")[0]) c->opt_wt_stores = atoi(getenv("LORADS_WT_STORES")) & WT_ALL;
    if (getenv("LORADS_FRONT_CHAIN") && getenv("LORADS_FRONT_CHAIN")[0]) c->opt_front_chain = atoi(getenv("LORADS_FRONT_CHAIN")) & FC_ALL;
    c->opt_spec_front = env_on("LORADS_SPEC_FRONT");
    c->opt_handover_on_front = env_on("LORADS_HANDOVER_ON_FRONT");
    if (getenv("LORADS_SPEC_WINDOW")) c->spec_window = std::max(1, std::min(8, atoi(getenv("LORADS_SPEC_WINDOW"))));
    c->opt_fold_avg = env_on("LORADS_FOLD_AVG");
    c->opt_tile_update = env_on("LORADS_TILE_UPDATE");
    c->opt_eval_diag = env_on("LORADS_EVAL_DIAG");
    c->opt_front_diag = env_on("LORADS_FRONT_DIAG");
    c->opt_dense_cache = env_on("LORADS_DENSE_CACHE");
    c->opt_bisect_lds = env_on("LORADS_BISECT_LDS");
    c->opt_fuse_eval = env_on("LORADS_FUSE_EVAL");
    c->opt_dense_rem = env_on("LORADS_DENSE_REM");
    c->opt_exact_refresh = env_set("LORADS_EXACT_REFRESH");
    c->opt_split_front = env_set("LORADS_SPLIT_FRONT");
    c->scal = (double *)c->ctrl;
    c->st = (CGState *)(c->ctrl + 64 * sizeof(double));
    c->h_scal = (double *)c->h_ctrl;
    c->h_st = (CGState *)(c->h_ctrl + 64 * sizeof(double));
    HC(hipMemset(c->lambda, 0, sizeof(double) * (size_t)std::max(c->m, 1)));
    HC(hipMemset(c->csum, 0, sizeof(double) * (size_t)(c->m + 2)));
    HC(hipMemset(c->q12, 0, sizeof(double) * (size_t)(2 * c->m + 2)));
    HC(hipMemset(c->scal, 0, sizeof(double) * 64));
    HC(hipMemset(c->ring_ab, 0, sizeof(double) * (size_t)2 * c->L));
    HC(hipMemset(c->st, 0, sizeof(CGState) * (size_t)std::max(2 * c->nb, 1)));
    if (M.alloc(&c->st_shadow, (size_t)std::max(2 * c->nb, 1))) return 1;
    HC(hipMemset(c->st_shadow, 0, sizeof(CGState) * (size_t)std::max(2 * c->nb, 1)));
    c->persist = new PersistPlan();
    c->opt_persist = env_on("LORADS_PERSIST");
    c->opt_persist_l2 = env_on("LORADS_PERSIST_L2");
    c->opt_persist_carry = env_on("LORADS_PERSIST_CARRY");
    c->opt_persist_rows = getenv("LORADS_PERSIST_ROWS") ? atoi(getenv("LORADS_PERSIST_ROWS")) : 0;
    c->opt_persist_linear = getenv("LORADS_PERSIST_MAP") && getenv("LORADS_PERSIST_MAP")[0] == 'l';
    c->lteam = new LTeamPlan();
    c->opt_lbfgs_team = env_on("LORADS_LBFGS_TEAM");
    c->opt_alm_fused_tail = env_on("LORADS_ALM_FUSED_TAIL");
    c->opt_alm_fold_cv = env_on("LORADS_ALM_FOLD_CV");
    c->opt_alm_sval_direct = env_on("LORADS_ALM_SVAL_DIRECT");
    if (env_set("LORADS_SHARED_GPU")) {
        int dev = 0;
        char bus[64] = "0";
        if (hipGetDevice(&dev) == hipSuccess) (void)hipDeviceGetPCIBusId(bus, sizeof(bus), dev);
        for (char *q = bus; *q; ++q) if (*q == ':' || *q == '.' || *q == '/') *q = '_';
        const std::string path = std::string("/tmp/lorads_gpu_") + bus + ".lock";
        c->shared_gpu_fd = open(path.c_str(), O_CREAT | O_RDWR, 0666);
    }
    HC(hipDeviceSynchronize());
    return 0;
}

}

extern "C" {

const char *lorads_hip_last_error(void) { return g_err.c_str(); }

int lorads_hip_create(const lorads_hip_problem *prob, lorads_hip_ctx **out) {
    *out = nullptr;
    int ndev = 0;
    if (hipGetDeviceCount(&ndev) != hipSuccess || ndev == 0)
        return fail_msg("no HIP device: the MI355X backend has no CPU fallback");
    if (prob->device >= 0) HC(hipSetDevice(prob->device));
    lorads_hip_ctx *c = new lorads_hip_ctx();
    if (ctx_init(c, prob)) { lorads_hip_destroy(c); return 1; }
    *out = c;
    return 0;
}

void lorads_hip_destroy(lorads_hip_ctx *c) {
    if (!c) return;
    if (c->stream) hipStreamSynchronize(c->stream);
    drain_events(c);
    for (auto &e : c->ev_pool) hipEventDestroy(e);
    graph_cache_free(c);
    if (c->persist) { c->persist->release(); delete c->persist; }
    if (c->lteam) { c->lteam->release(); delete c->lteam; }
    c->cert.release();
    c->rnd.release();
    c->spectral.release();
    c->primal.release();
    c->cuts.release();
    c->bounds.release();
    c->topk.release();
    c->kcut.release();
    c->stable.release();
    c->bisect.release();
    c->factor_mem.release();
// ... 751 lines not shown
    return 0;
}

int lorads_hip_persist_plan(lorads_hip_ctx *c, int64_t out[8]) {
    spec_touch(c);
    const bool ok = c->persist && persist_ready(c, 800);
    const PersistPlan *P = c->persist;
    out[0] = ok ? (int64_t)P->tag : -1;
    out[1] = ok && P->xcd_map ? 1 : 0;
    out[2] = ok ? P->g_max : 0;
    out[3] = ok ? P->nsub_max : 0;
    out[4] = ok ? P->ssz_max : 0;
    out[5] = ok ? P->occ : 0;
    out[6] = ok ? P->ncu : 0;
    out[7] = ok && c->opt_persist_l2 ? 1 : 0;
    return 0;
}

int lorads_hip_persist_set_tag(lorads_hip_ctx *c, uint32_t tag) {
    spec_touch(c);
    if (!c->persist || !c->persist->valid) return fail_msg("persist_set_tag: no plan of the one-launch ADMM iteration is valid");
    PersistPlan &P = *c->persist;
    c->pend.flush(c);
    HC(hipStreamSynchronize(c->stream));
    HC(hipMemset(P.gran, 0, sizeof(unsigned long long) * std::max<size_t>(P.gran_words, 1)));
    P.tag = tag;
    return 0;
}

int lorads_hip_launch_count(lorads_hip_ctx *c, int64_t *n) {
    spec_touch(c);
    *n = c->n_launch;
    return 0;
}

int lorads_hip_memory_stats(int64_t stats[4]) {
    for (int i = 0; i < 4; ++i) stats[i] = g_mem_live[i].load();
    return 0;
}

int lorads_hip_lbfgs_team_stats(lorads_hip_ctx *c, int64_t stats[4]) {
    spec_touch(c);
    const bool ok = c->lteam && c->lteam->valid;
    stats[0] = c->lteam ? c->lteam->launches : 0;
    stats[1] = ok ? 1 : 0;
    stats[2] = ok ? c->lteam->grid : 0;
    stats[3] = ok ? c->lteam->np : 0;
    return 0;
}

int lorads_hip_persist_stamps(lorads_hip_ctx *c, int32_t enable, uint64_t ticks[16]) {
    spec_touch(c);
    c->pend.flush(c);
    HC(hipStreamSynchronize(c->stream));
    for (int i = 0; i < 16; ++i) ticks[i] = 0;
    if (c->persist && c->persist->valid && c->persist->stamps && c->persist_stamps) {
        HC(hipMemcpy(c->persist->h_stamps, c->persist->stamps, sizeof(unsigned long long) * 16, hipMemcpyDeviceToHost));
        for (int i = 0; i < 16; ++i) ticks[i] = c->persist->h_stamps[i];
        HC(hipMemset(c->persist->stamps, 0, sizeof(unsigned long long) * 16));
    }
    c->persist_stamps = enable != 0;
    return 0;
}

int lorads_hip_presolve_stats(lorads_hip_ctx *c, int64_t stats[2]) {
    spec_touch(c);
    stats[0] = c->n_dev_patterns;
    stats[1] = c->n_checked_patterns;
    return 0;
}

int lorads_hip_spec_front_stats(lorads_hip_ctx *c, int64_t out[4]) {
    if (!c || !out) return fail_msg("spec_front_stats: bad argument");
    out[0] = c->n_spec_enq; out[1] = c->n_spec_adopt; out[2] = c->n_spec_discard; out[3] = c->n_spec_blocked;
    return 0;
}

int lorads_hip_handover_stats(lorads_hip_ctx *c, int64_t out[2]) {
    if (!c || !out) return fail_msg("handover_stats: bad argument");
    out[0] = c->n_handover_front; out[1] = c->n_handover_alone;
    return 0;
}

int lorads_hip_row_deal_stats(lorads_hip_ctx *c, int32_t k, int out[3]) {
    if (!c || !out) return fail_msg("row_deal_stats: bad argument");
    if (k < 0 || k >= c->nb) return fail_msg("bad block");
    const RowDeal rd = row_deal_of(c, c->blk[k]);
    out[0] = rd.rpw; out[1] = rd.grid; out[2] = c->row_deal_cus;
    return 0;
}

int lorads_hip_wt_stores(lorads_hip_ctx *c, int *mask) {
    if (!c || !mask) return fail_msg("wt_stores: bad argument");
    *mask = c->opt_wt_stores;
    return 0;
}

int lorads_hip_front_chain(lorads_hip_ctx *c, int *mask, int *eff) {
    if (!c || !mask) return fail_msg("front_chain: bad argument");
    *mask = c->opt_front_chain;
    if (eff) {
        *eff = 0;
        for (const Block &B : c->blk)
            if (B.front_cw && c->opt_front_lds && (B.r + 15) / 16 <= 3) *eff = c->opt_front_chain;
    }
    return 0;
}

int lorads_hip_dense_plan(lorads_hip_ctx *c, int32_t k, int64_t out[16]) {
    if (!c || !out) return fail_msg("dense_plan: bad argument");
    if (k < 0 || k >= c->nb) return fail_msg("bad block");
    for (int i = 0; i < 16; ++i) out[i] = 0;
    const Block &B = c->blk[k];
    if (!B.dense_c && !B.dense_a) return 0;
    out[0] = B.npad; out[1] = B.ksplit_b;
    for (int col0 = 0; col0 < B.r && out[2] < 4; col0 += 128) {
        const DenseTiles tl = dense_tiles(B.r, col0, c->opt_dense_rem);
        int64_t *o = out + 3 + 3 * out[2]++;
        o[0] = col0; o[1] = tl.nt; o[2] = tl.rem;
    }
    out[15] = !B.wj_for ? 0 : B.wj_for == c->U + B.off ? 1 : B.wj_for == c->V + B.off ? 2 : 3;
    return 0;
}

int lorads_hip_graph_stats(lorads_hip_ctx *c, int64_t stats[4]) {
    spec_touch(c);
    stats[0] = c->graphs ? c->graphs->n_capture : 0;
    stats[1] = c->graphs ? c->graphs->n_replay : 0;
    stats[2] = c->graphs ? (int64_t)c->graphs->map.size() : 0;
    stats[3] = graph_ok(c) ? 1 : 0;
    return 0;
}

int lorads_hip_algorithmic_bytes(lorads_hip_ctx *c, int32_t k, double *mv, double *cg) {
    spec_touch(c);
    if (k < 0 || k >= c->nb) return fail_msg("bad block");
    const Block &B = c->blk[k];
    const double F = 8.0 * (double)B.n * (double)B.rl;
    *mv = 4 * F + 32.0 * B.na + 16.0 * B.nrow;
    *cg = *mv + 9 * F;
    return 0;
}

}

#include "lanczos.inc"
#include "postsolve.inc"
#include "solution.inc"
#include "rounding.inc"
#include "kcut.inc"
#include "stable.inc"
#include "bisect.inc"
#include "spectral.inc"
#include "primal.inc"
#include "select.inc"
#include "cuts.inc"
#include "bounds.inc"
#include "topk.inc"
```

### lorads_amd/csrc/hip/sweep.inc

```
#define LAUNCH_LDS(kern, grid, lds, ...)                                                             \
    do {                                                                                             \
        const int grid__ = (int)(grid);                                                              \
        if (c->pend.must_flush()) c->pend.flush(c);                                                  \
        if (grid__ > 0) { ++c->n_launch; hipLaunchKernelGGL(kern, dim3(grid__), dim3(TPB), (size_t)(lds), c->stream, __VA_ARGS__); } \
    } while (0)
#define LAUNCH(kern, grid, ...) LAUNCH_LDS(kern, grid, 0, __VA_ARGS__)
#include "pending.inc"

struct Shape {
    int lg, v2, ns;
};
inline Shape shape_for(int r) {
    Shape s;
    s.v2 = use_v2(r);
    s.lg = lg_for(r);
    const int w = s.v2 ? 2 : 1;
    s.ns = (r + s.lg * w - 1) / (s.lg * w);
    return s;
}
#define NS_SWITCH(LGV, V2V, ns, ...)                                     \
    switch (ns) {                                                        \
    case 1: { constexpr int LG_ = LGV; constexpr bool V2_ = V2V; constexpr int NS_ = 1; __VA_ARGS__; } break; \
    case 2: { constexpr int LG_ = LGV; constexpr bool V2_ = V2V; constexpr int NS_ = 2; __VA_ARGS__; } break; \
    case 3: { constexpr int LG_ = LGV; constexpr bool V2_ = V2V; constexpr int NS_ = 3; __VA_ARGS__; } break; \
    case 4: { constexpr int LG_ = LGV; constexpr bool V2_ = V2V; constexpr int NS_ = 4; __VA_ARGS__; } break; \
    case 5: { constexpr int LG_ = LGV; constexpr bool V2_ = V2V; constexpr int NS_ = 5; __VA_ARGS__; } break; \
    case 6: { constexpr int LG_ = LGV; constexpr bool V2_ = V2V; constexpr int NS_ = 6; __VA_ARGS__; } break; \
    case 7: { constexpr int LG_ = LGV; constexpr bool V2_ = V2V; constexpr int NS_ = 7; __VA_ARGS__; } break; \
    default: { constexpr int LG_ = LGV; constexpr bool V2_ = V2V; constexpr int NS_ = 8; __VA_ARGS__; } break; \
    }
#define SHAPE_DISPATCH(sh, ...)                                   \
    do {                                                          \
        if ((sh).v2) { NS_SWITCH(8, true, (sh).ns, __VA_ARGS__) }        \
        else if ((sh).lg == 8) { NS_SWITCH(8, false, (sh).ns, __VA_ARGS__) } \
        else if ((sh).lg == 32) { NS_SWITCH(32, false, (sh).ns, __VA_ARGS__) } \
        else { NS_SWITCH(64, false, (sh).ns, __VA_ARGS__) }              \
    } while (0)

void pairdots(lorads_hip_ctx *c, const Pattern &P, const double *X, const double *Y, int r, double *T, Guard g) {
    if (P.ne == 0) return;
    const Shape sh = shape_for(r);
    const int grid = nblocks_for((size_t)P.ne, TPB / sh.lg);
    SHAPE_DISPATCH(sh, LAUNCH((k_pairdots<LG_, V2_, NS_>), grid, P.ne, P.erow, P.ecol, X, Y, r, T, g));
}
int spmm(lorads_hip_ctx *c, const Block &B, const Pattern &P, const double *X, int mode, const double *xin, const double *rhs,
         double rho, double *out, double *part, Guard g, const double *dense_add = nullptr) {
    const Shape sh = shape_for(B.r);
    const int grid = nblocks_for((size_t)B.n, TPB / sh.lg);
    SHAPE_DISPATCH(sh, LAUNCH((k_spmm2<LG_, V2_, NS_, false>), grid, B.n, P.adj_ptr, P.adj_col, P.adj_dyn, P.adj_sval, P.S, (const double *)nullptr, X,
                              B.r, mode, xin, rhs, ds_rho(c, rho), out, (double *)nullptr, part, (double *)nullptr, g, dense_add));
    return grid;
}
struct DiagOnFly {
    bool on = false;
    WArgs wa{};
    int wmode = 0;
    CGState *reset = nullptr;
    int nreset = 0;
    Deferred d{};
};
int spmm_front(lorads_hip_ctx *c, const Block &B, const Pattern &P, const double *X, const double *xin, double rho, double *rhs_out,
               double *out, double *part, double *part_b, Guard g, const DiagOnFly &of = DiagOnFly{}) {
    const Shape sh = shape_for(B.r);
    const int grid = nblocks_for((size_t)B.n, TPB / sh.lg);
    if (of.on) {
        SHAPE_DISPATCH(sh, LAUNCH((k_spmm2<LG_, V2_, NS_, true>), grid, B.n, P.adj_ptr, P.adj_col, P.adj_dyn, P.adj_sval, P.S,
                                  (const double *)nullptr, X, B.r, 0, xin, (const double *)nullptr, ds_rho(c, rho), out, rhs_out, part, part_b, g,
                                  (const double *)nullptr, (const double *)B.gdiag, B.w_uv, (const int *)B.rc_con, B.rc_w,
                                  (const double *)B.diag_a, of.wa, of.wmode, of.reset, of.nreset, of.d));
        return grid;
    }
    SHAPE_DISPATCH(sh, LAUNCH((k_spmm2<LG_, V2_, NS_, true>), grid, B.n, P.adj_ptr, P.adj_col, P.adj_dyn, P.adj_sval, P.S,
                              (const double *)(B.diag_only ? nullptr : P.S2), X, B.r, 0, xin, (const double *)nullptr, ds_rho(c, rho), out, rhs_out,
                              part, part_b, g, (const double *)nullptr, (const double *)(B.diag_only ? B.gdiag : nullptr),
                              B.diag_only ? B.w_uv : (double *)nullptr));
    return grid;
}
RowDeal row_deal_of(const lorads_hip_ctx *c, const Block &B) {
    const size_t n = (size_t)std::max(B.n, 0);
    if (c->opt_row_deal == 0 || &B == &c->merged) return RowDeal{32, nblocks_for(n, 32)};
    if (c->opt_row_deal > 0) {
        const int rpw = nblocks_for(n, c->opt_row_deal) <= c->maxpart ? c->opt_row_deal : 32;
        return RowDeal{rpw, nblocks_for(n, rpw)};
    }
    return row_deal(n, c->row_deal_cus);
}
int spmm_cw(lorads_hip_ctx *c, const Block &B, const double *w, const double *X, int mode, const double *xin, const double *rhs,
            double *out, double *part, Guard g, const Cg0Args *cg0 = nullptr) {
    const Shape sh = shape_for(B.r);
    const int grid = nblocks_for((size_t)B.n, TPB / sh.lg);
    const RowDeal rd = sh.lg == 8 ? row_deal_of(c, B) : RowDeal{TPB / sh.lg, grid};
    if (cg0) {
        if (!B.cell_w || !sh.v2 || mode != OP_CG) { c->launch_err = "CG iteration 0 in the operator: no kernel form for this cone"; return 0; }
        if (B.cell_w == 8) {
            NS_SWITCH(8, true, sh.ns, LAUNCH((k_spmm_ell<LG_, V2_, NS_, 8, true>), rd.grid, B.n, rd.rpw, B.cadj_ptr, B.cadj_col, B.cadj_con, B.cadj_a,
                                             B.cell_col, B.cell_con, B.cell_a, w, X, B.r, mode, xin, rhs, (double *)nullptr, part, g, *cg0))
        } else {
            NS_SWITCH(8, true, sh.ns, LAUNCH((k_spmm_ell<LG_, V2_, NS_, 16, true>), rd.grid, B.n, rd.rpw, B.cadj_ptr, B.cadj_col, B.cadj_con, B.cadj_a,
                                             B.cell_col, B.cell_con, B.cell_a, w, X, B.r, mode, xin, rhs, (double *)nullptr, part, g, *cg0))
        }
        return rd.grid;
    }
    if (B.cell_w && (mode == OP_CG || mode == OP_RES)) {
        Cg0Args wo{};
        wo.wt = c->opt_wt_stores;
        if (B.cell_w == 8)
            SHAPE_DISPATCH(sh, LAUNCH((k_spmm_ell<LG_, V2_, NS_, 8>), rd.grid, B.n, rd.rpw, B.cadj_ptr, B.cadj_col, B.cadj_con, B.cadj_a, B.cell_col,
                                      B.cell_con, B.cell_a, w, X, B.r, mode, xin, rhs, out, part, g, wo));
        else
            SHAPE_DISPATCH(sh, LAUNCH((k_spmm_ell<LG_, V2_, NS_, 16>), rd.grid, B.n, rd.rpw, B.cadj_ptr, B.cadj_col, B.cadj_con, B.cadj_a, B.cell_col,
                                      B.cell_con, B.cell_a, w, X, B.r, mode, xin, rhs, out, part, g, wo));
        return rd.grid;
    }
    SHAPE_DISPATCH(sh, LAUNCH((k_spmm<LG_, V2_, NS_, true>), grid, B.n, B.cadj_ptr, B.cadj_col, B.cadj_con, w, X, B.r, mode, xin, rhs,
                              0.0, out, part, g, (const double *)nullptr, B.cadj_a));
    return grid;
}
bool cw_quad(lorads_hip_ctx *c, const Block &B) {
    return c->opt_cw_quad && use_v2(B.r) && B.r <= 48 && B.ca_ell > 8 && B.ca_ell <= 16;
}
int cw(lorads_hip_ctx *c, const Block &B, const double *X, const double *Y, double scale, double *w_out, double *cv, int mode,
       double *vec, Guard g, ResArgs ra = ResArgs{}) {
    if (B.nrow == 0) return 0;
    const Shape sh = shape_for(B.r);
    const int grid = nblocks_for((size_t)B.nrow, TPB / 64);
    const InitArgs ia = c->pend.take_init_on(g);
    const Deferred d = c->pend.take_check_behind(g);
    if (cw_quad(c, B)) {
        const int ns4 = (B.r + 7) / 8;
        NS_SWITCH(4, true, ns4, LAUNCH((k_cw<LG_, V2_, NS_, true>), grid, B.nrow, B.a_ptr, B.ca_row, B.ca_val, B.ca_col, X, Y, B.r,
                                       scale, w_out, cv, mode, B.row_idx, vec, g, B.ca_ell, ia, ra, d));
        return grid;
    }
    SHAPE_DISPATCH(sh, LAUNCH((k_cw<LG_, V2_, NS_>), grid, B.nrow, B.a_ptr, B.ca_row, B.ca_val, B.ca_col, X, Y, B.r, scale,
                              w_out, cv, mode, B.row_idx, vec, g, B.ca_ell, ia, ra, d));
    return grid;
}
struct DenseTiles { int nt, rem; };
static inline DenseTiles dense_tiles(int r, int col0, bool use_rem) {
    const int cols = std::min(r - col0, 128);
    DenseTiles t{(cols + 15) / 16, 0};
    if (cols % 16 >= 1 && cols % 16 <= 4 && t.nt >= 2 && use_rem) { t.rem = cols % 16; t.nt -= 1; }
    return t;
}
int dense_cx(lorads_hip_ctx *c, const Block &B, const double *X, double *W, Guard g, const double *M = nullptr) {
    c->pend.flush(c);
    if (!M) M = B.Cfull;
    if (B.ksplit_b <= 0) return 1;
    {
        const int gx = B.npad / 32, ks = B.ksplit_b, krange = B.npad / ks;
        double *dst = ks == 1 ? W : B.Wpart;
        for (int col0 = 0; col0 < B.r; col0 += 128) {
            const DenseTiles tl = dense_tiles(B.r, col0, c->opt_dense_rem);
            const int nt = tl.nt, rem = tl.rem;
#define DCXB(NTV, RV) hipLaunchKernelGGL((k_dense_cx_b<NTV, 4, RV>), dim3(gx, ks), dim3(TPB), 0, c->stream, B.n, B.npad, krange, M, X, B.r, dst, g, col0)
#define DCXR(NTV)                                  \
    switch (rem) {                                 \
    case 1: DCXB(NTV, 1); break;                   \
    case 2: DCXB(NTV, 2); break;                   \
    case 3: DCXB(NTV, 3); break;                   \
    case 4: DCXB(NTV, 4); break;                   \
    default: DCXB(NTV, 0); break;                  \
    }
            switch (nt) {
            case 1: DCXR(1); break;
            case 2: DCXR(2); break;
            case 3: DCXR(3); break;
            case 4: DCXR(4); break;
            case 5: DCXR(5); break;
            case 6: DCXR(6); break;
            case 7: DCXR(7); break;
            default: DCXR(8); break;
            }
#undef DCXR
#undef DCXB
        }
// ... 49 lines not shown

int op_diag(lorads_hip_ctx *c, const Block &B, const double *V, int mode, const double *xin, const double *rhs, double *out,
            double *part, Guard g, double *dot_out = nullptr) {
    const Shape sh = shape_for(B.r);
    const int grid = nblocks_for((size_t)B.n, TPB / sh.lg);
    Carry cy{};
    cy.ia = c->pend.take_init_on(g);
    if (!cy.ia.st) cy.d = c->pend.take_check_on(g);
    const DirArgs da = c->pend.take_on_op_diag(c, mode, xin, g, TPB / sh.lg);
    SHAPE_DISPATCH(sh, LAUNCH((k_op_diag<LG_, V2_, NS_>), grid, B.n, B.gdiag, V, B.r, mode, xin, rhs, out, part, g, cy, da, dot_out));
    return grid;
}
int op_entry(lorads_hip_ctx *c, const Block &B, const double *V, int mode, const double *xin, const double *rhs, double *out,
             double *part, Guard g) {
    const Shape sh = shape_for(B.r);
    if (B.bip_rows[0] && c->opt_entry_bip) {
        const int g0 = nblocks_for((size_t)B.bip_n[0], TPB / sh.lg), g1 = nblocks_for((size_t)B.bip_n[1], TPB / sh.lg);
        if (g0 + g1 <= c->maxpart) {
            SHAPE_DISPATCH(sh, LAUNCH((k_op_entry_bip<LG_, V2_, NS_, 0>), g0, B.bip_n[0], (const int *)B.bip_rows[0], B.pa.adj_ptr, B.pa.adj_col,
                                      B.pa.adj_e, B.gentry, B.bip_we, V, B.r, mode, xin, rhs, out, part, 0, g));
            SHAPE_DISPATCH(sh, LAUNCH((k_op_entry_bip<LG_, V2_, NS_, 1>), g1, B.bip_n[1], (const int *)B.bip_rows[1], B.pa.adj_ptr, B.pa.adj_col,
                                      B.pa.adj_e, B.gentry, B.bip_we, V, B.r, mode, xin, rhs, out, part, g0, g));
            return g0 + g1;
        }
    }
    const int grid = nblocks_for((size_t)B.n, TPB / sh.lg);
    SHAPE_DISPATCH(sh, LAUNCH((k_op_entry<LG_, V2_, NS_>), grid, B.n, B.pa.adj_ptr, B.pa.adj_col, B.pa.adj_e, B.gentry, V, B.r, mode, xin,
                              rhs, out, part, g));
    return grid;
}
int obj_partials(lorads_hip_ctx *c, const Block &B, const double *X, const double *Y, double *part, Guard g,
                 double *stage_tail = nullptr) {
    if (B.nc == 0) return 0;
    if (B.dense_c) {
        if (dense_cx(c, B, Y, B.Wd, g)) c->launch_err = "dense GEMM: no kernel form for this rank";
        const size_t len = (size_t)B.n * B.r;
        const int grid = grid1d(len);
        LAUNCH(k_dot, grid, len, X, B.Wd, part, g);
        return grid;
    }
    const Shape sh = shape_for(B.r);
    const int grid = stage_tail ? 2048 : std::min(nblocks_for((size_t)B.nc, TPB / sh.lg), 2048);
    SHAPE_DISPATCH(sh, LAUNCH((k_obj<LG_, V2_, NS_>), grid, B.nc, B.c_row, B.c_col, B.c_val, X, Y, B.r, part, g, stage_tail));
    return grid;
}

void constr_val(lorads_hip_ctx *c, Block &B, const double *X, const double *Y, double scale, double *cv, int mode, double *vec,
                Guard g) {
    if (B.nrow == 0) return;
    const bool uv = (X == c->U + B.off && Y == c->V + B.off);
    if (B.use_cw) {
        cw(c, B, X, Y, scale, uv ? B.w_uv : (double *)nullptr, cv, mode, vec, g);
        if (uv) B.t_uv_valid = true;
        return;
    }
    double *T = uv ? B.T : B.T2;
    pairdots(c, B.pa, X, Y, B.r, T, g);
    if (uv) B.t_uv_valid = true;
    LAUNCH(k_cv, nblocks_for((size_t)B.nrow, TPB / 8), B.nrow, B.a_ptr, B.a_e, B.a_val, T, scale, cv, mode, B.row_idx, vec, g);
    dense_constr_fix(c, B, X, Y, scale, cv, vec, g);
}
void sval(lorads_hip_ctx *c, const Pattern &P, bool with_c, int mode, const WArgs &wa, Guard g, CGState *reset = nullptr,
          int nreset = 0, const double *w2 = nullptr, const int *econ = nullptr) {
    if (P.ne == 0 && !reset) return;
    const Deferred d = c->pend.take_check_behind(g);
    LAUNCH(k_sval, std::max(1, nblocks_for((size_t)P.ne, TPB)), P.ne, P.e_ptr, econ ? econ : P.e_con, P.e_val,
           with_c ? P.cbase : nullptr, mode, wa, P.S, g, reset, nreset, w2, w2 ? P.S2 : (double *)nullptr, d);
}

int wsum(lorads_hip_ctx *c, Block &B, Guard g, double *part_ww = nullptr) {
    const InitArgs ia = c->pend.take_init_on(g);
    double rho_dual = 0.0;
    const int dual_on = c->pend.take_dual_used(&rho_dual) ? 1 : 0;
    const int grid = nblocks_for((size_t)B.nrow, TPB / 8);
    CGState *reset = c->spec.reset;
    const int nreset = c->spec.nreset;
    c->spec.reset = nullptr; c->spec.nreset = 0;
    LAUNCH(k_wsum, grid, B.nrow, B.cs_w, (const double *)B.w_contrib, B.w_op, g, ia, dual_on, ds_rho_dual(c, rho_dual), c->m, (const double *)c->b,
           (const double *)c->csum, c->lambda, part_ww, reset, nreset);
    return grid;
}

int apply_operator(lorads_hip_ctx *c, Block &B, const double *V, const double *x, int mode, const double *rhs, double *out,
                   double *part, Guard g, double *part_ww = nullptr, const Cg0Args *cg0 = nullptr) {
    const bool samp = c->prof && c->prof_target == 0 && c->prof_every < (1 << 20) && (c->n_matvec % c->prof_every == 0) &&
                      c->ev_next + 3 <= c->ev_pool.size();
    hipEvent_t e0 = nullptr, e1 = nullptr, e2 = nullptr;
    if (samp) {
        e0 = c->ev_pool[c->ev_next++]; e1 = c->ev_pool[c->ev_next++];
        hipEventRecord(e0, c->stream);
    }
    int grid;
    if (B.diag_only) {
        const bool is_uv = (x == c->U + B.off && V == c->V + B.off) || (x == c->V + B.off && V == c->U + B.off);
        double *dots = !B.w_op ? (double *)nullptr : (mode == OP_CG && !is_uv) ? B.w_op : (mode == OP_RES && is_uv) ? B.w_uv : (double *)nullptr;
        grid = op_diag(c, B, V, mode, x, rhs, out, part, g, dots);
        if (dots && dots == B.w_uv) B.t_uv_valid = true;
    } else if (B.entry_only) {
        grid = op_entry(c, B, V, mode, x, rhs, out, part, g);
    } else if (B.use_cw) {
        const bool is_uv = (x == c->U + B.off && V == c->V + B.off) || (x == c->V + B.off && V == c->U + B.off);
        const double *w = B.w_uv;
        if (B.w0_ready && mode == OP_CG && x == c->cr + B.off) {
            wsum(c, B, g, part_ww);
            w = B.w_op;
            B.t_uv_valid = false;
        } else if (!(is_uv && B.t_uv_valid)) {
            cw(c, B, x, V, 1.0, is_uv ? B.w_uv : B.w_op, (double *)nullptr, (int)CV_SET, (double *)nullptr, g);
            w = is_uv ? B.w_uv : B.w_op;
            B.t_uv_valid = is_uv;
        }
        B.w0_ready = false;
        grid = spmm_cw(c, B, w, V, mode, x, rhs, out, part, g, cg0);
    } else {
        const bool is_uv = (x == c->U + B.off && V == c->V + B.off) || (x == c->V + B.off && V == c->U + B.off);
        if (!(is_uv && B.t_uv_valid)) {
            pairdots(c, B.pa, x, V, B.r, B.T, g);
            B.t_uv_valid = is_uv;
        }
        if (B.has_gram) {
            LAUNCH(k_sgram, nblocks_for((size_t)B.pa.ne, TPB / 8), B.pa.ne, B.g_ptr, B.g_col, B.g_val, B.T, B.pa.S, g);
        } else {
            LAUNCH(k_cv, nblocks_for((size_t)B.nrow, TPB / 8), B.nrow, B.a_ptr, B.a_e, B.a_val, B.T, 1.0, B.wtmp, (int)CV_SET,
                   B.row_idx, (double *)nullptr, g);
            dense_constr_fix(c, B, x, V, 1.0, B.wtmp, (double *)nullptr, g);
            WArgs wa{};
            wa.w = B.wtmp;
            sval(c, B.pa, false, W_COMPACT, wa, g);
            if (B.dense_a) dense_part(c, B, V, W_COMPACT, wa, 1.0, false, g);
        }
        if (samp) { e2 = c->ev_pool[c->ev_next++]; hipEventRecord(e2, c->stream); }
        grid = spmm(c, B, B.pa, V, mode, x, rhs, 0.0, out, part, g, B.dense_a ? B.Wd : (const double *)nullptr);
    }
    if (samp) {
        hipEventRecord(e1, c->stream);
        c->timed_mv.push_back({e0, e1});
        if (e2) c->timed_sp.push_back({e2, e1});
    }
    c->n_matvec++;
    return grid;
}

void drain_events(lorads_hip_ctx *c) {
    for (auto &pr : c->timed_mv) {
        float ms = 0;
        hipEventSynchronize(pr.second);
        hipEventElapsedTime(&ms, pr.first, pr.second);
        c->ms_samp += ms; c->n_samp++;
        c->samp_ms.push_back(ms);
    }
    for (auto &pr : c->timed_sp) {
        float ms = 0;
        hipEventElapsedTime(&ms, pr.first, pr.second);
        c->ms_samp_spmm += ms; c->n_samp_spmm++;
    }
    c->timed_mv.clear();
    c->timed_sp.clear();
    c->ev_next = 0;
}

bool constr_by_recurrence(lorads_hip_ctx *c, const Block &B) {
    return (B.use_cw || (B.diag_only && B.w_uv && B.w_op && B.diag_row)) && !c->opt_exact_refresh && &B != &c->merged;
}

bool fused_front(lorads_hip_ctx *c, const Block &B) {
    return ((B.use_cw && B.pu.S2) || B.diag_only) && !B.dense_c && !B.dense_a && !c->opt_split_front && B.pu.ne > 0;
}

bool front_cw_ok(lorads_hip_ctx *c, const Block &B) {
    return c->opt_front_cw && B.front_cw && fused_front(c, B) && B.use_cw && B.cell_w && use_v2(B.r) && &B != &c->merged;
}

struct FrontSample {
    lorads_hip_ctx *c;
    hipEvent_t e0 = nullptr, e1 = nullptr;
    explicit FrontSample(lorads_hip_ctx *c_) : c(c_) {
        const bool samp = c->prof && c->prof_target == 1 && c->prof_every < (1 << 20) && (c->n_front % c->prof_every == 0) &&
                          c->ev_next + 2 <= c->ev_pool.size();
        c->n_front++;
        if (samp) { e0 = c->ev_pool[c->ev_next++]; e1 = c->ev_pool[c->ev_next++]; hipEventRecord(e0, c->stream); }
    }
    void done() { if (e0) { hipEventRecord(e1, c->stream); c->timed_mv.push_back({e0, e1}); } }
};

struct Solve {
    Block *B;
    double *x;
    const double *V;
    CGState *st;
    Guard front;
    size_t len;
    int gv;
    int tile = 0, tile_w = 0;
};

FrontCwArgs front_cw_args(lorads_hip_ctx *c, const Block &B, double rho, int wmode) {
    FrontCwArgs A{};
    A.fc_ptr = B.fc_ptr; A.fc_col = B.fc_col; A.fc_val = B.fc_val; A.sl_ptr = B.cadj_ptr; A.sl_col = B.cadj_col; A.sl_con = B.cadj_con;
    A.sl_a = B.cadj_a; A.ell_col = B.cell_col; A.ell_con = B.cell_con; A.ell_a = B.cell_a; A.ell_dst = B.cell_dst; A.sl_dst = B.cadj_dst; A.csum = c->csum; A.b = c->b;
    A.lambda = c->lambda; A.cv = B.cv; A.w_uv = B.w_uv; A.row_idx = B.row_idx_identity ? nullptr : B.row_idx; A.rho = ds_rho(c, rho);
    A.wmode = wmode;
    A.contrib = B.w_contrib;
    A.wt = c->opt_wt_stores;
    return A;
}
int launch_front_cw(lorads_hip_ctx *c, const Solve &s, const FrontCwArgs &A, Guard g, Deferred d, const HandoverArgs *ho = nullptr) {
    Block &B = *s.B;
    double *r = c->cr + B.off, *rhs = c->rhs + B.off;
    double *pA = part_slot(c, 18), *pB = part_slot(c, 1);
    const RowDeal rd = row_deal_of(c, B);
    const int grid = rd.grid;
    const int ns = (B.r + 15) / 16;
    const bool keep = c->pend.set_dual_used(false);
    FrontSample fs(c);
    FrontCwHoArgs AH{};
    const int lead = ho ? 1 : 0;
    if (ho) { static_cast<FrontCwArgs &>(AH) = A; AH.ho = *ho; AH.ho.lead = lead; }
    const int fc = c->opt_front_chain & FC_ALL;
#define FC_SWITCH(...)                                             \
    do { switch (fc) {                                             \
    case 0: { constexpr int FC_ = 0; __VA_ARGS__; } break;         \
    case 1: { constexpr int FC_ = 1; __VA_ARGS__; } break;         \
    case 2: { constexpr int FC_ = 2; __VA_ARGS__; } break;         \
    default: { constexpr int FC_ = 3; __VA_ARGS__; } break;        \
    } } while (0)
#define FCW(EWV, HO, AV) NS_SWITCH(8, true, ns, LAUNCH((k_front_cw<NS_, EWV, 0, HO>), grid + lead, B.n, rd.rpw, AV, s.V, B.r, (const double *)s.x, r, rhs, pA, pB, g, d))
#define FCWL(NSV, EWV, HO, AV) FC_SWITCH(LAUNCH_LDS((k_front_cw<NSV, EWV, 4, HO, FC_>), grid + lead, sizeof(double2) * 32 * 4 * NSV * 8, B.n, rd.rpw, AV, s.V, B.r, (const double *)s.x, r, rhs, pA, pB, g, d))
#define FRONT(HO, AV)                                                                                                    \
    if (c->opt_front_lds && ns <= 3) {                                                                                   \
        if (B.cell_w == 8) { if (ns == 1) FCWL(1, 8, HO, AV); else if (ns == 2) FCWL(2, 8, HO, AV); else FCWL(3, 8, HO, AV); }     \
        else { if (ns == 1) FCWL(1, 16, HO, AV); else if (ns == 2) FCWL(2, 16, HO, AV); else FCWL(3, 16, HO, AV); }                \
    } else if (B.cell_w == 8) { FCW(8, HO, AV) } else { FCW(16, HO, AV) }
    if (ho) { FRONT(true, AH) } else { FRONT(false, A) }
#undef FRONT
#undef FCWL
#undef FCW
#undef FC_SWITCH
    fs.done();
    c->pend.set_dual_used(keep);
    return grid;
}
void front_cw_started(lorads_hip_ctx *c, const Solve &s, int grid, double tol) {
    s.B->w0_ready = true;
    c->pend.post_init(c, s.st, part_slot(c, 18), grid, part_slot(c, 1), grid, tol, s.front);
}
bool front_carries_dual(const lorads_hip_ctx *c, const Solve &s, int wmode) {
    return c->pend.dual_rides(s.front) && wmode == W_ADMM && c->nb == 1;
}
bool spec_front_adopt(lorads_hip_ctx *c, const Solve &s, double rho, double tol, CGState *reset, int nreset);

void solve_front(lorads_hip_ctx *c, const Solve &s, double rho, double tol, CGState *reset = nullptr, int nreset = 0) {
    Block &B = *s.B;
    double *r = c->cr + B.off, *p = c->cp + B.off, *rhs = c->rhs + B.off;
    double *pA = part_slot(c, 18), *pB = part_slot(c, 1);
    WArgs wa{};
    wa.csum = c->csum; wa.b = c->b; wa.lambda = c->lambda; wa.cv = B.cv; wa.row_idx = B.row_idx_identity ? nullptr : B.row_idx; wa.rho = ds_rho(c, rho);
    B.w0_ready = false;
    if (front_cw_ok(c, B)) {
        if (!B.t_uv_valid) {
            cw(c, B, s.x, s.V, 1.0, B.w_uv, (double *)nullptr, (int)CV_SET, (double *)nullptr, s.front);
            B.t_uv_valid = true;
        }
        if (spec_front_adopt(c, s, rho, tol, reset, nreset)) return;
        FrontCwArgs A = front_cw_args(c, B, rho, c->virt_refresh ? W_ADMM_V : W_ADMM);
        c->virt_refresh = false;
        A.reset = reset; A.nreset = nreset;
        if (front_carries_dual(c, s, A.wmode)) {
            A.rho_dual = ds_rho_dual(c, c->pend.use_dual());
            A.dual_on = 1;
        }
        const Deferred d = c->pend.take_check_behind(s.front);
        front_cw_started(c, s, launch_front_cw(c, s, A, s.front, d), tol);
        return;
    }
    if (fused_front(c, B)) {
        if (B.use_cw && !B.t_uv_valid) {
            cw(c, B, s.x, s.V, 1.0, B.w_uv, (double *)nullptr, (int)CV_SET, (double *)nullptr, s.front);
            B.t_uv_valid = true;
        }
        int wmode = W_ADMM;
        if (c->virt_refresh && (B.use_cw || B.diag_only)) {
            wmode = W_ADMM_V;
            wa.w = B.w_uv;
            if (B.diag_only) { wa.drow = B.diag_row; wa.da = B.diag_a; }
        }
        c->virt_refresh = false;
        const bool carry_dual = c->pend.dual_rides(s.front) && wmode == W_ADMM && B.pu.e_con_own && B.nrow == c->m && B.pu.n_owned == c->m && c->nb == 1;
        const int *econ = B.pu.e_con;
        if (carry_dual) {
            wa.lambda_out = c->lambda_alt;
            wa.rho_dual = ds_rho_dual(c, c->pend.take_dual());
            econ = B.pu.e_con_own;
        }
        const bool onfly = B.diag_only && B.rc_w > 0 && B.w_uv && c->opt_front_diag && &B != &c->merged;
        DiagOnFly of{};
        if (onfly) {
            of.on = true; of.wa = wa; of.wmode = wmode; of.reset = reset; of.nreset = nreset;
            of.d = c->pend.take_check_behind(s.front);
        } else {
            sval(c, B.pu, true, wmode, wa, s.front, reset, nreset, B.use_cw ? B.w_uv : (const double *)nullptr, econ);
        }
        FrontSample fs(c);
        const int nf = spmm_front(c, B, B.pu, s.V, s.x, rho, rhs, r, pA, pB, s.front, of);
        fs.done();
        if (carry_dual) std::swap(c->lambda, c->lambda_alt);
        if (B.diag_only && B.w_uv) B.t_uv_valid = true;
        c->pend.post_init(c, s.st, pA, nf, pB, nf, tol, s.front);
        return;
    }
    sval(c, B.pu, true, W_ADMM, wa, s.front, reset, nreset);
    if (B.dense_a && B.wj_for != s.V) dense_cache_fill(c, B, s.V, s.front);
    if (B.dense_c || B.dense_a) dense_part(c, B, s.V, W_ADMM, wa, 1.0, true, s.front);
    const int nb1 = spmm(c, B, B.pu, s.V, OP_RHS, nullptr, nullptr, rho, rhs, pB, s.front, (B.dense_c || B.dense_a) ? B.Wd : nullptr);
    const int na = apply_operator(c, B, s.V, s.x, OP_RES, rhs, r, pA, s.front);
    c->pend.post_init(c, s.st, pA, na, pB, nb1, tol, s.front);
}
bool cg0_rule(lorads_hip_ctx *c, const Block &B) {
    return front_cw_ok(c, B) && B.nrow > 0 && nblocks_for((size_t)B.nrow, TPB / 8) <= c->maxpart;
}
void solve_iter_body(lorads_hip_ctx *c, const Solve &s, int k, double tol, int maxit, bool fold_avg = false) {
    Block &B = *s.B;
    double *r = c->cr + B.off, *p = k == 0 ? c->cr + B.off : c->cp + B.off, *Q = c->cQ + B.off;
    double *pA = part_slot(c, 0), *pC = part_slot(c, 2);
    const Guard g{&s.st->done, s.front.need};
    const bool rec = constr_by_recurrence(c, B) && B.t_uv_valid;
    const int nw = !rec ? 0 : B.diag_only ? B.n : B.nrow;
    const bool v2 = (s.len & 1) == 0 && (((uintptr_t)s.x | (uintptr_t)r | (uintptr_t)p | (uintptr_t)Q) & 15) == 0;
    const int store_r = (k % 20 != 0 || !c->opt_lazy_scalars) ? 1 : 0;
    const double *avg_other = fold_avg ? s.V : (const double *)nullptr;
    double *avg_out = fold_avg ? c->R + B.off : (double *)nullptr;
    if (fold_avg) c->avg_folded = true;
    const bool v2_avg = v2 && (!fold_avg || (((uintptr_t)avg_other | (uintptr_t)avg_out) & 15) == 0);
    const bool rule0 = k == 0 && B.w0_ready && cg0_rule(c, B);
    double *pW = rule0 ? part_slot(c, 20) : (double *)nullptr;
    const int nww = rule0 ? nblocks_for((size_t)B.nrow, TPB / 8) : 0;
    const bool fuse0 = rule0 && c->opt_fuse_cg0 && v2_avg;
    Cg0Args u{};
    u.wt = c->opt_wt_stores;
    if (fuse0) {
        u.st = s.st; u.part_ww = pW; u.nww = nww; u.x = s.x; u.r = r; u.store_r = store_r;
        u.w_acc = rec ? B.w_uv : (double *)nullptr; u.w_p = B.w_op; u.nw = nw; u.shadow = shadow_of(c, s.st);
        u.avg_other = avg_other; u.avg_out = avg_out;
    }
    const int npq = apply_operator(c, B, s.V, p, OP_CG, nullptr, Q, fuse0 ? pC : pA, g, pW, fuse0 ? &u : (const Cg0Args *)nullptr);
    int nrr = npq;
    if (!fuse0) {
        if (v2_avg)
            LAUNCH(k_cg_update<true>, s.gv, s.len, s.st, pA, npq, s.x, r, p, Q, pC, g, rec ? B.w_uv : (double *)nullptr,
                   (const double *)B.w_op, nw, shadow_of(c, s.st), store_r, avg_other, avg_out, s.tile, s.tile_w, (const double *)pW, nww);
        else
            LAUNCH(k_cg_update<false>, s.gv, s.len, s.st, pA, npq, s.x, r, p, Q, pC, g, rec ? B.w_uv : (double *)nullptr,
                   (const double *)B.w_op, nw, shadow_of(c, s.st), store_r, avg_other, avg_out, s.tile, s.tile_w, (const double *)pW, nww);
        nrr = s.gv;
    }
    B.t_uv_valid = rec;
    if (B.wj_for == s.x) B.wj_for = nullptr;
    c->merged.t_uv_valid = false;
    c->pend.post_check(c, s.st, pC, nrr, tol, maxit, g);
}
void solve_iter_tail(lorads_hip_ctx *c, const Solve &s, int k, double tol, int maxit, bool runs_for_sure = false) {
    Block &B = *s.B;
    double *r = c->cr + B.off, *p = c->cp + B.off, *rhs = c->rhs + B.off;
    double *pA = part_slot(c, 19);
    const Guard g{&s.st->done, s.front.need};
    if (k % 20 == 0) {
        const bool was_valid = B.t_uv_valid;
        if (k > 0) B.t_uv_valid = false;
        const int nr = apply_operator(c, B, s.V, s.x, OP_RES, rhs, r, pA, g);
        if (!was_valid && !runs_for_sure) B.t_uv_valid = false;
        if (c->opt_lazy_scalars && B.diag_only && c->opt_fuse_dir) {
            c->pend.post_dir(Pending::Dir{DIR_RESTART, s.st, r, p, s.len, s.gv, pA, nr, g});
        } else if (c->opt_lazy_scalars) {
            LAUNCH(k_cg_dir, s.gv, s.len, s.st, (int)DIR_RESTART, r, p, g, Deferred{}, (const double *)pA, nr);
        } else {
            LAUNCH(k_cg_check, 1, s.st, (int)CHK_RESTART, pA, nr, ds_tol(c, tol), ds_maxit(c, maxit), g);
            LAUNCH(k_cg_dir, s.gv, s.len, s.st, (int)DIR_RESTART, r, p, g);
        }
    } else if (c->opt_lazy_scalars && B.diag_only && c->opt_fuse_dir) {
        c->pend.post_dir(Pending::Dir{DIR_BETA, s.st, r, p, s.len, s.gv, nullptr, 0, g});
    } else {
        const Deferred d = c->pend.take_check_of(s.st);
        LAUNCH(k_cg_dir, s.gv, s.len, s.st, (int)DIR_BETA, r, p, g, d);
    }
}
void solve_iters(lorads_hip_ctx *c, const Solve &s, int k0, int k1, double tol, int maxit, bool fold_avg_last = false) {
    for (int k = k0; k < k1; ++k) {
        if (k > k0) solve_iter_tail(c, s, k - 1, tol, maxit);
        solve_iter_body(c, s, k, tol, maxit, fold_avg_last && k == k1 - 1);
    }
}
void refresh_after_solve(lorads_hip_ctx *c, Block &B, const int *need) {
    if (constr_by_recurrence(c, B) && B.t_uv_valid && B.nrow > 0) {
        const Deferred d = c->pend.take_check_behind(Guard{nullptr, need});
        LAUNCH(k_refresh_w, nblocks_for((size_t)B.nrow, TPB), B.nrow, (const double *)B.w_uv, B.cv, B.row_idx, c->csum,
               Guard{nullptr, need}, d, B.diag_only ? (const int *)B.diag_row : (const int *)nullptr,
               B.diag_only ? (const double *)B.diag_a : (const double *)nullptr);
        return;
    }
    constr_val(c, B, c->U + B.off, c->V + B.off, 1.0, B.cv, CV_DELTA, c->csum, Guard{nullptr, need});
}

void flush_final(lorads_hip_ctx *c);
bool spec_front_enqueue(lorads_hip_ctx *c, double rho, const HandoverArgs *ho = nullptr);
int enqueue_publish(lorads_hip_ctx *c, size_t word0, size_t nwords, const double *front_rho = nullptr, bool *front_carried = nullptr) {
    if (c->sx_pending && (word0 > SX_WORD || word0 + nwords < SX_WORD + 4)) {
        const size_t w1 = std::max(word0 + nwords, (size_t)SX_WORD + 4);
        word0 = std::min(word0, (size_t)SX_WORD);
        nwords = w1 - word0;
    }
    int sep_with_obj = 0;
    SepExtra ex{};
    const bool sep = !c->final_pending && c->pend.take_sep(4, &sep_with_obj, &ex);
    c->pend.flush(c);
    ++c->pub_seq;
    if (sep) {
        LAUNCH(k_publish_sep, 1, (const double *)c->sepbuf, c->scal, sep_with_obj, ex.n, ex.p[0], ex.p[1], ex.p[2],
               ex.p[3], (const unsigned long long *)c->ctrl + word0, (int)nwords, (unsigned long long *)c->h_ctrl_dev + word0,
               c->h_flag_dev, c->seq_dev);
    } else if (c->final_pending) {
        const HandoverArgs H{c->final_args, (const unsigned long long *)c->ctrl + word0, (unsigned long long *)c->h_ctrl_dev + word0,
                             (int)nwords, c->h_flag_dev, c->seq_dev, 0};
        const bool own = (const double *)H.src == H.fa.out;
        if (front_rho && c->opt_handover_on_front && own && spec_front_enqueue(c, *front_rho, &H)) {
            *front_carried = true;
            c->final_pending = false;
            ++c->n_handover_front;
            return 0;
// ... 74 lines not shown
    s.gv = std::min(grid1d(s.len), 512);
    if (B.diag_only && c->opt_tile_update) {
        const int rows = TPB / shape_for(B.r).lg, g = nblocks_for((size_t)B.n, rows);
        if (g <= c->maxpart && rows * B.r >= TPB / 2) { s.gv = g; s.tile = rows * B.r; s.tile_w = rows; }
    }
    return s;
}

bool spec_front_ok(lorads_hip_ctx *c) {
    if (!c->opt_spec_front || !c->use_publish || c->ar || c->nb != 1 || !c->opt_lazy_scalars || !c->lambda_alt) return false;
    if (c->prof && c->prof_every < (1 << 20)) return false;
    return front_cw_ok(c, c->blk[0]) && !c->blk[0].is_lp;
}
bool spec_front_enqueue(lorads_hip_ctx *c, double rho, const HandoverArgs *ho) {
    Block &B = c->blk[0];
    if (!B.t_uv_valid || c->pend.dual_owed()) return false;
    const Solve s = make_solve(c, 0, 0, nullptr);
    FrontCwArgs A = front_cw_args(c, B, rho, W_ADMM);
    A.dual_on = 1;
    A.rho_dual = ds_rho_dual(c, rho);
    launch_front_cw(c, s, A, Guard{nullptr, &c->st[2 * c->nb - 1].done}, Deferred{}, ho);
    c->spec.live = true; c->spec.dual_seen = false;
    c->spec.rho = rho; c->spec.rho_dual = rho; c->spec.wmode = W_ADMM; c->spec.epoch = c->spec_epoch;
    ++c->n_spec_enq;
    return true;
}
bool spec_front_adopt(lorads_hip_ctx *c, const Solve &s, double rho, double tol, CGState *reset, int nreset) {
    if (!c->spec.live) return false;
    c->spec.live = false;
    Block &B = *s.B;
    const bool ok = s.st == c->st && reset && !c->par_mode && c->spec.epoch == c->spec_epoch && memcmp(&rho, &c->spec.rho, sizeof(double)) == 0 &&
                    c->spec.dual_seen && c->pend.dual_owed_at(c->spec.rho_dual) && !c->virt_refresh &&
                    c->spec.wmode == W_ADMM && front_carries_dual(c, s, W_ADMM) && B.t_uv_valid && c->opt_lazy_scalars &&
                    B.spec[0] >= 1;
    if (!ok) { ++c->n_spec_discard; return false; }
    ++c->n_spec_adopt;
    c->pend.use_dual();
    c->virt_refresh = false;
    c->spec.reset = reset; c->spec.nreset = nreset;
    c->n_front++;
    front_cw_started(c, s, row_deal_of(c, B).grid, tol);
    return true;
}

void enqueue_lp_sweep(lorads_hip_ctx *c, Block &B, double rho, CGState *st, Guard g) {
    c->pend.flush(c);
    LpArgs A;
    A.ncols = B.n; A.nlev = B.lp_nlev; A.lvl_ptr = B.lp_lvl_ptr; A.lvl_cols = B.lp_lvl_cols; A.ptr = B.lp_ptr; A.grow = B.lp_grow;
    A.a = B.lp_a; A.nrm2sq = B.lp_nrm2sq; A.cobj = B.lp_cobj; A.cv = B.lp_cv; A.U = c->U + B.off; A.V = c->V + B.off;
    A.csum = c->csum; A.b = c->b; A.lambda = c->lambda; A.rho = ds_rho(c, rho);
    B.t_uv_valid = false;
    if (B.lp_nlev <= 1) {
        LAUNCH(k_lp_sweep_flat, nblocks_for((size_t)B.n, TPB), A, g);
        hipLaunchKernelGGL(k_lp_done, dim3(1), dim3(1), 0, c->stream, st, g);
    } else {
        LAUNCH(k_lp_sweep, 1, A, st, g);
    }
}
void lp_col_values(lorads_hip_ctx *c, Block &B, const double *X, const double *Y, Guard g) {
    if (!B.is_lp || B.n == 0) return;
    LAUNCH(k_lp_cv, nblocks_for((size_t)B.n, TPB), B.n, B.lp_ptr, B.lp_a, X + B.off, Y + B.off, B.lp_cv, g);
}

void enqueue_sweep(lorads_hip_ctx *c, int first, int resume_iter, double rho, double tol, int maxit, bool eval_follows) {
    c->virt_refresh = false;
    for (int stg = first; stg < 2 * c->nb; ++stg) {
        const int k = stg / 2, half = stg % 2;
        const int *need = stg == 0 ? nullptr : &c->st[stg - 1].done;
        Solve s = make_solve(c, k, half, need);
        Block &B = *s.B;
        if (B.is_lp) {
            if (half == 0) enqueue_lp_sweep(c, B, rho, c->st + stg, Guard{nullptr, need});
            continue;
        }
        if (stg == first && resume_iter >= 0) {
            const int more = std::max(2, std::min(resume_iter, 16));
            if (resume_iter > 0) solve_iter_tail(c, s, resume_iter - 1, tol, maxit, true);
            solve_iters(c, s, resume_iter, std::min(resume_iter + more, maxit), tol, maxit);
        } else {
            const bool fresh0 = stg == 0 && resume_iter < 0 && 2 * c->nb - 1 <= TPB;
            solve_front(c, s, rho, tol, fresh0 ? c->st + 1 : nullptr, fresh0 ? 2 * c->nb - 1 : 0);
            const bool fold = eval_follows && stg == 2 * c->nb - 1 && c->nb == 1 && B.use_cw && c->opt_lazy_scalars &&
                              c->opt_fold_avg && B.nrow > 0 && nblocks_for((size_t)B.nrow, TPB / 64) <= c->maxpart;
            solve_iters(c, s, 0, std::min(B.spec[half], maxit), tol, maxit, fold);
        }
        if (eval_follows && stg == 2 * c->nb - 1) {
            if (B.use_cw) {
                const bool exact_now = (c->n_sweeps % 32) == 31;
                if (!(constr_by_recurrence(c, B) && B.t_uv_valid) || exact_now)
                    cw(c, B, c->U + B.off, c->V + B.off, 1.0, B.w_uv, (double *)nullptr, (int)CV_SET, (double *)nullptr,
                       Guard{nullptr, &s.st->done});
                B.t_uv_valid = true;
            } else if (!B.diag_only && !B.entry_only) {
                pairdots(c, B.pa, c->U + B.off, c->V + B.off, B.r, B.T, Guard{nullptr, &s.st->done});
                B.t_uv_valid = true;
            }
        } else if (eval_follows && c->nb == 1 && stg == 0 && c->opt_lazy_scalars && constr_by_recurrence(c, B) && B.t_uv_valid &&
                   fused_front(c, B) && (B.use_cw || B.diag_only)) {
            c->virt_refresh = true;
        } else {
            if (stg == 2 * c->nb - 1 && (c->n_sweeps % 32) == 31) B.t_uv_valid = false;
            refresh_after_solve(c, B, &s.st->done);
        }
    }
}

int first_unfinished(lorads_hip_ctx *c, int first) {
    for (int stg = first; stg < 2 * c->nb; ++stg)
        if (c->h_st[stg].done == 0) return stg;
    return -1;
}

void flush_final(lorads_hip_ctx *c) {
    if (!c->final_pending) return;
    const EvalFinalArgs &fa = c->final_args;
    LAUNCH(k_eval_final, 1, fa.part_v, fa.part_d, fa.np, fa.out, fa.g, fa.obj_part, fa.nobj);
    c->final_pending = false;
}
int enqueue_eval(lorads_hip_ctx *c, int pair, const int *need, bool with_obj = true) {
    flush_final(c);
    const Guard g{nullptr, need};
    const bool vec = shard_vec(c);
    Block *Dc = solo(c);
    Block *D1 = (pair == LORADS_HIP_PAIR_UV && !vec && c->opt_eval_diag && Dc && Dc->diag_only && Dc->rc_w > 0 && Dc->nrow == c->m &&
                 c->m > 0 && Dc->w_uv && !c->avg_folded && !Dc->dense_c) ? Dc : nullptr;
    if (D1) {
    } else if (pair == LORADS_HIP_PAIR_UV && c->avg_folded && need) {
        c->avg_folded = false;
    } else if (pair == LORADS_HIP_PAIR_UV) {
        c->avg_folded = false;
        const Deferred d = c->pend.take_check_behind(g);
        LAUNCH(k_average, grid1d(c->all_elem), c->all_elem, c->U, c->V, c->R, g, d);
    }
    Block *S1 = solo(c);
    if (S1 && (S1->nrow != c->m || S1->dense_c)) S1 = c->nb == 1 ? S1 : nullptr;
    const bool single = (S1 && S1->nrow == c->m) || (c->nb == 1 && c->blk[0].nrow == c->m);
    bool any_dense_a = false;
    for (auto &B0 : c->blk) any_dense_a = any_dense_a || B0.dense_a;
    const bool fold_res = single && !vec && c->m > 0 && !any_dense_a;
    c->ls_np = 0;
    double *dst = vec ? c->cstage : c->csum;
    std::vector<Block *> cones;
    if (S1) cones.push_back(S1);
    else for (auto &B0 : c->blk) cones.push_back(&B0);
    if (vec && c->ar_fast_all < 0) {
        double v[2] = {(c->opt_ar_fast && c->nb == 1 && !c->blk[0].dense_c && c->blk[0].nc > 0 && !c->blk[0].is_lp) ? 1.0 : 0.0, 1.0};
        c->pend.flush(c);
        HC(hipStreamSynchronize(c->stream));
        if (c->ar(c->ar_user, v, 2, 0)) return fail_msg("allreduce hook failed");
        c->ar_fast_all = v[0] == v[1] ? 1 : 0;
    }
    const bool ar_fast = vec && with_obj && c->ar_fast_all == 1 && cones.size() == 1;
    if ((!single || vec) && !(ar_fast && c->stage_clean)) LAUNCH(k_zero, grid1d((size_t)c->m), (size_t)c->m, dst, g);
    bool first_obj = true;
    const bool fold_obj = (c->nb == 1 || S1) && !vec;
    int nobj = 0, nres = 0;
    for (Block *bp : cones) {
        Block &B = *bp;
        if (D1 == &B && fold_res) {
            const Deferred d = c->pend.take_check_behind(g);
            const Shape sh = shape_for(B.r);
            nres = nblocks_for((size_t)B.n, TPB / sh.lg);
            SHAPE_DISPATCH(sh, LAUNCH((k_eval_diag<LG_, V2_, NS_>), nres, B.n, (const double *)(c->U + B.off), (const double *)(c->V + B.off),
                                      c->R + B.off, B.r, B.rc_w, (const int *)B.rc_con, (const double *)B.diag_a,
                                      B.row_idx_identity ? (const int *)nullptr : (const int *)B.row_idx, B.cv, c->csum,
                                      (const double *)c->b, (const double *)c->lambda, part_slot(c, 8), part_slot(c, 9), g, d));
        } else if (fold_res && B.use_cw && with_obj && fold_obj && c->opt_fuse_eval && cw_quad(c, B) && B.nc > 0 && !B.dense_c &&
// ... 351 lines not shown
```

### lorads_amd/host.py

```python
import ctypes as C
import os

import numpy as np

_HERE = os.path.dirname(os.path.abspath(__file__))
LIB_DIR = os.path.join(_HERE, "lib")
DEV_LIB = os.path.join(LIB_DIR, "liblorads_hip_dev.so")

PAIR_RR, PAIR_UV = 0, 1
MAT_R, MAT_U, MAT_V, MAT_GRAD = 0, 1, 2, 3
VEC_LAMBDA, VEC_CONSTR_SUM, VEC_Q1, VEC_Q2 = 0, 1, 2, 3

_dp = C.POINTER(C.c_double)
_ip = C.POINTER(C.c_int)
ALLREDUCE_FN = C.CFUNCTYPE(C.c_int, C.c_void_p, C.c_void_p, C.c_int, C.c_int)


class BackendStruct(C.Structure):
    _fields_ = [
        ("ctx", C.c_void_p),
        ("name", C.c_char_p),
        ("init_constr", C.CFUNCTYPE(C.c_int, C.c_void_p, C.c_int)),
        ("alm_cal_grad", C.CFUNCTYPE(C.c_int, C.c_void_p, C.c_double, _dp)),
        ("lbfgs_direction", C.CFUNCTYPE(C.c_int, C.c_void_p, C.c_int)),
# ... 614 lines not shown
        buf, n = (C.c_double * cap)(), C.c_int()
        _check(lib.lorads_hip_profile_samples(ctx, buf, cap, C.byref(n)), "profile_samples")
        return [buf[i] for i in range(min(cap, n.value))]

    def hip_time_operator(self, reps):
        lib, ctx = self._hip()
        ms = C.c_double()
        lib.lorads_hip_time_operator.argtypes = [C.c_void_p, C.c_int, _dp]
        rc = lib.lorads_hip_time_operator(ctx, int(reps), C.byref(ms))
        if rc:
            lib.lorads_hip_last_error.restype = C.c_char_p
            raise RuntimeError("time_operator: %s" % (lib.lorads_hip_last_error() or b"?").decode())
        return ms.value

    def hip_ubench(self, which, reps):
        lib, ctx = self._hip()
        if not hasattr(lib, "lorads_hip_ubench"):
            raise RuntimeError("ubench: not in the product library (attach the session to host.DEV_LIB)")
        lib.lorads_hip_ubench.argtypes = [C.c_void_p, C.c_int, C.c_int, _dp]
        ms = C.c_double()
        rc = lib.lorads_hip_ubench(ctx, int(which), int(reps), C.byref(ms))
        if rc:
            lib.lorads_hip_last_error.restype = C.c_char_p
            raise RuntimeError("ubench: %s" % (lib.lorads_hip_last_error() or b"?").decode())
        return ms.value

    def hip_algorithmic_bytes(self, blk=0):
        lib, ctx = self._hip()
        a, b = C.c_double(), C.c_double()
        _check(lib.lorads_hip_algorithmic_bytes(ctx, blk, C.byref(a), C.byref(b)), "algorithmic_bytes")
        return a.value, b.value

    def hip_dual_infeasibility(self, tol=1e-2, ncv=40, max_restarts=600):
        lib, ctx = self._hip()
        lib.lorads_hip_dual_infeasibility.argtypes = [C.c_void_p, C.c_double, C.c_int, C.c_int, _dp, _dp, _ip]
        nb = self.nblk
        v, lm, mv = C.c_double(), (C.c_double * max(nb, 1))(), C.c_int()
        _check(lib.lorads_hip_dual_infeasibility(ctx, tol, ncv, max_restarts, C.byref(v), lm, C.byref(mv)), "dual_infeasibility")
        return v.value, [lm[i] for i in range(nb)], mv.value

    def hip_certificate(self, src, tol=1e-8, ncv=40, max_restarts=600):
        lib, ctx = self._hip()
        lib.lorads_hip_certificate.argtypes = [C.c_void_p, C.c_int, C.c_double, C.c_int, C.c_int, _dp, _dp, _dp, _dp]
        nb, m = self.nblk, self.m
        out, lm = (C.c_double * 10)(), (C.c_double * max(nb, 1))()
        res, lam = (C.c_double * max(m, 1))(), (C.c_double * max(m, 1))()
        _check(lib.lorads_hip_certificate(ctx, int(src), tol, ncv, max_restarts, out, lm, res, lam), "certificate")
        return (np.array(out[:10]), np.array(lm[:nb]), np.array(res[:m]), np.array(lam[:m]))

    def hip_get_slack(self, blk):
        lib, ctx = self._hip()
        i32p = C.POINTER(C.c_int32)
        lib.lorads_hip_get_slack.argtypes = [C.c_void_p, C.c_int, C.POINTER(C.c_int64), i32p, i32p, _dp]
        nnz = C.c_int64()
        _check(lib.lorads_hip_get_slack(ctx, int(blk), C.byref(nnz), None, None, None), "get_slack")
        row, col, val = np.zeros(nnz.value, dtype=np.int32), np.zeros(nnz.value, dtype=np.int32), np.zeros(nnz.value)
        _check(lib.lorads_hip_get_slack(ctx, int(blk), C.byref(nnz), row.ctypes.data_as(i32p), col.ctypes.data_as(i32p),
                                        val.ctypes.data_as(_dp)), "get_slack")
        return row, col, val

    def hip_block_image(self, blk=0):
        lib, ctx = self._hip()
        out = (C.c_int64 * 16)()
        lib.lorads_hip_block_image.argtypes = [C.c_void_p, C.c_int, C.POINTER(C.c_int64)]
        _check(lib.lorads_hip_block_image(ctx, blk, out), "block_image")
        keys = ["n", "rank", "nrow", "na", "nc", "pattern_a", "pattern_union", "dense_c", "dense_a", "diag_only", "entry_only", "use_cw",
                "has_gram", "front_cw", "slot_width", "bip_rows0"]
        return dict(zip(keys, [int(out[i]) for i in range(16)]))

    def hip_spec_front_stats(self):
        lib, ctx = self._hip()
        out = (C.c_int64 * 4)()
        lib.lorads_hip_spec_front_stats.argtypes = [C.c_void_p, C.POINTER(C.c_int64)]
        _check(lib.lorads_hip_spec_front_stats(ctx, out), "spec_front_stats")
        return dict(zip(["enqueued", "adopted", "discarded", "blocked"], [int(out[i]) for i in range(4)]))

    def hip_handover_stats(self):
        lib, ctx = self._hip()
        out = (C.c_int64 * 2)()
        lib.lorads_hip_handover_stats.argtypes = [C.c_void_p, C.POINTER(C.c_int64)]
        _check(lib.lorads_hip_handover_stats(ctx, out), "handover_stats")
        return dict(zip(["on_front", "alone"], [int(out[i]) for i in range(2)]))

    def hip_row_deal_stats(self, blk=0):
        lib, ctx = self._hip()
        out = (C.c_int * 3)()
        lib.lorads_hip_row_deal_stats.argtypes = [C.c_void_p, C.c_int32, C.POINTER(C.c_int)]
        _check(lib.lorads_hip_row_deal_stats(ctx, blk, out), "row_deal_stats")
        return dict(zip(["rpw", "grid", "ncu"], [int(out[i]) for i in range(3)]))

    def hip_wt_stores(self):
        lib, ctx = self._hip()
        out = C.c_int(-1)
        lib.lorads_hip_wt_stores.argtypes = [C.c_void_p, C.POINTER(C.c_int)]
        _check(lib.lorads_hip_wt_stores(ctx, C.byref(out)), "wt_stores")
        return int(out.value)

    def hip_front_chain(self, effective=False):
        lib, ctx = self._hip()
        out, eff = C.c_int(-1), C.c_int(-1)
        lib.lorads_hip_front_chain.argtypes = [C.c_void_p, C.POINTER(C.c_int), C.POINTER(C.c_int)]
        _check(lib.lorads_hip_front_chain(ctx, C.byref(out), C.byref(eff)), "front_chain")
        return int(eff.value if effective else out.value)

    def hip_dense_plan(self, blk=0):
        lib, ctx = self._hip()
        out = (C.c_int64 * 16)()
        lib.lorads_hip_dense_plan.argtypes = [C.c_void_p, C.c_int32, C.POINTER(C.c_int64)]
        _check(lib.lorads_hip_dense_plan(ctx, blk, out), "dense_plan")
        return dict(npad=int(out[0]), ksplit=int(out[1]), launches=[tuple(int(out[3 + 3 * i + j]) for j in range(3)) for i in range(int(out[2]))],
                    kept=("", "U", "V", "other")[int(out[15])])

    def hip_graph_stats(self):
        lib, ctx = self._hip()
        out = (C.c_int64 * 4)()
        lib.lorads_hip_graph_stats.argtypes = [C.c_void_p, C.POINTER(C.c_int64)]
        _check(lib.lorads_hip_graph_stats(ctx, out), "graph_stats")
        return dict(zip(["captured", "replayed", "held", "enabled"], [int(out[i]) for i in range(4)]))

    def hip_persist_stats(self):
        lib, ctx = self._hip()
        out = (C.c_int64 * 6)()
        lib.lorads_hip_persist_stats.argtypes = [C.c_void_p, C.POINTER(C.c_int64)]
        _check(lib.lorads_hip_persist_stats(ctx, out), "persist_stats")
        return dict(zip(["iterations", "available", "workgroups", "rows", "column_steps", "lds_bytes"], [int(out[i]) for i in range(6)]))

    def hip_persist_plan(self):
        lib, ctx = self._hip()
        out = (C.c_int64 * 8)()
        lib.lorads_hip_persist_plan.argtypes = [C.c_void_p, C.POINTER(C.c_int64)]
        _check(lib.lorads_hip_persist_plan(ctx, out), "persist_plan")
        return dict(zip(["tag", "xcd_map", "team", "sub_teams", "sub_team", "occ", "ncu", "allow_l2"], [int(out[i]) for i in range(8)]))

    def hip_persist_set_tag(self, tag):
        lib, ctx = self._hip()
        lib.lorads_hip_persist_set_tag.argtypes = [C.c_void_p, C.c_uint32]
        _check(lib.lorads_hip_persist_set_tag(ctx, int(tag)), "persist_set_tag")

    def hip_launch_count(self):
        lib, ctx = self._hip()
        out = C.c_int64(0)
        lib.lorads_hip_launch_count.argtypes = [C.c_void_p, C.POINTER(C.c_int64)]
        _check(lib.lorads_hip_launch_count(ctx, C.byref(out)), "launch_count")
        return int(out.value)

    @staticmethod
    def hip_memory_stats(libpath=None):
        lib = C.CDLL(libpath or os.path.join(LIB_DIR, "liblorads_hip.so"))
        out = (C.c_int64 * 4)()
        lib.lorads_hip_memory_stats.argtypes = [C.POINTER(C.c_int64)]
        _check(lib.lorads_hip_memory_stats(out), "memory_stats")
        return dict(zip(("device_allocations", "device_bytes", "pinned_allocations", "pinned_bytes"), [int(out[i]) for i in range(4)]))

    def hip_lbfgs_team_stats(self):
        lib, ctx = self._hip()
        out = (C.c_int64 * 4)()
        lib.lorads_hip_lbfgs_team_stats.argtypes = [C.c_void_p, C.POINTER(C.c_int64)]
        _check(lib.lorads_hip_lbfgs_team_stats(ctx, out), "lbfgs_team_stats")
        return dict(zip(("launches", "available", "workgroups", "pairs"), [int(out[i]) for i in range(4)]))

    def hip_persist_stamps(self, enable=True):
        lib, ctx = self._hip()
        out = (C.c_uint64 * 16)()
        lib.lorads_hip_persist_stamps.argtypes = [C.c_void_p, C.c_int, C.POINTER(C.c_uint64)]
        _check(lib.lorads_hip_persist_stamps(ctx, 1 if enable else 0, out), "persist_stamps")
        return [int(out[i]) for i in range(16)]
# ... 537 lines not shown
```

Baseline: 10340.

## Precompute front weight records in the CG iteration-0 kernel for the V-half front

When the U-half solve runs a single fused CG iteration and a V-half front follows, the CG0 SpMM kernel now also writes a packed (m1, w) double2 record per row. That record is computed from csum, b, lambda, cv and the updated weight. The next front kernel reads this record instead of gathering five arrays and recomputing the multiplier for each nonzero, which cuts repeated indirect loads. Several host-side guards (rho, launch count, dual state, parity) decide when the record is valid. This costs an extra buffer, extra stores in the CG0 kernel and more template instantiations.

```diff
diff --git a/include/lorads_hip.h b/include/lorads_hip.h
--- a/include/lorads_hip.h
+++ b/include/lorads_hip.h
@@ -125,6 +125,7 @@
 int lorads_hip_sync(lorads_hip_ctx *ctx);
 int lorads_hip_spec_front_stats(lorads_hip_ctx *ctx, int64_t out[4]);
 int lorads_hip_handover_stats(lorads_hip_ctx *ctx, int64_t out[2]);
+int lorads_hip_front_wrec_stats(lorads_hip_ctx *ctx, int64_t out[2]);
 int lorads_hip_row_deal_stats(lorads_hip_ctx *ctx, int32_t block, int out[3]);
 int lorads_hip_wt_stores(lorads_hip_ctx *ctx, int *mask);
 int lorads_hip_front_chain(lorads_hip_ctx *ctx, int *mask, int *effective);
diff --git a/lorads_amd/csrc/hip/build.inc b/lorads_amd/csrc/hip/build.inc
--- a/lorads_amd/csrc/hip/build.inc
+++ b/lorads_amd/csrc/hip/build.inc
@@ -439,7 +439,8 @@
                     for (int i = 0; i < B.n; ++i)
                         for (int sl = 0; sl < B.cell_w && ptr[i] + sl < ptr[i + 1]; ++sl) dste[(size_t)i * B.cell_w + sl] = dstc[ptr[i] + sl];
                     if (M.upload(&B.fc_ptr, hpC.adj_ptr) || M.upload(&B.fc_col, hpC.adj_col) || M.upload(&B.fc_val, fval) ||
-                        M.upload(&B.cadj_dst, dstc) || M.upload(&B.cell_dst, dste) || M.alloc(&B.w_contrib, (size_t)hb.nrow * csw))
+                        M.upload(&B.cadj_dst, dstc) || M.upload(&B.cell_dst, dste) || M.alloc(&B.w_contrib, (size_t)hb.nrow * csw) ||
+                        M.alloc(&B.wrec, (size_t)2 * std::max(hb.nrow, 1)))
                         return 1;
                     HC(hipMemset(B.w_contrib, 0, sizeof(double) * std::max<size_t>((size_t)hb.nrow * csw, 1)));
                     B.cs_w = csw;
diff --git a/lorads_amd/csrc/hip/dev.inc b/lorads_amd/csrc/hip/dev.inc
--- a/lorads_amd/csrc/hip/dev.inc
+++ b/lorads_amd/csrc/hip/dev.inc
@@ -49,19 +49,22 @@
             else LAUNCH((k_spmm_ell<8, true, 3, 16>), rd.grid, B.n, rd.rpw, B.cadj_ptr, B.cadj_col, B.cadj_con, B.cadj_a, B.cell_col, B.cell_con,
                         B.cell_a, (const double *)B.w_op, V, B.r, (int)OP_CG, U, (const double *)nullptr, Q, part_slot(c, 0), NOGUARD);
             break;
-        case 30: case 31: case 33: case 34: {
+        case 30: case 31: case 33: case 34: case 35: case 36: {
             if (!B.front_cw) return fail_msg("ubench: cone without the one-kernel front's data");
             FrontCwArgs A{};
             A.fc_ptr = B.fc_ptr; A.fc_col = B.fc_col; A.fc_val = B.fc_val; A.sl_ptr = B.cadj_ptr; A.sl_col = B.cadj_col; A.sl_con = B.cadj_con;
             A.sl_a = B.cadj_a; A.ell_col = B.cell_col; A.ell_con = B.cell_con; A.ell_a = B.cell_a; A.ell_dst = B.cell_dst; A.sl_dst = B.cadj_dst;
             A.csum = c->csum; A.b = c->b; A.lambda = c->lambda; A.cv = B.cv; A.w_uv = B.w_op;
             A.row_idx = B.row_idx_identity ? nullptr : B.row_idx; A.rho = 1.0; A.wmode = W_ADMM;
-            A.contrib = (which == 30 || which == 33) ? B.w_contrib : (double *)nullptr;
+            A.contrib = (which == 30 || which == 33 || which == 35) ? B.w_contrib : (double *)nullptr;
             A.wt = c->opt_wt_stores;
+            if (which >= 35) A.wrec = (const double2 *)Q;
+            if (which >= 35 && it == -3) hipLaunchKernelGGL(k_fill, dim3(64), dim3(TPB), 0, c->stream, (size_t)2 * B.nrow, 1.0, Q);
             const size_t lds = sizeof(double2) * 32 * 4 * 3 * 8;
-#define UB_FRONT(EWV, FCV) LAUNCH_LDS((k_front_cw<3, EWV, 4, false, FCV>), rd.grid, lds, B.n, rd.rpw, A, V, B.r, U, r, rhs, part_slot(c, 0), part_slot(c, 1), NOGUARD, Deferred{})
-            if (which < 33) { if (B.cell_w == 8) UB_FRONT(8, 0); else UB_FRONT(16, 0); }
-            else { if (B.cell_w == 8) UB_FRONT(8, FC_ALL); else UB_FRONT(16, FC_ALL); }
+#define UB_FRONT(EWV, FCV, WRV) LAUNCH_LDS((k_front_cw<3, EWV, 4, false, FCV, WRV>), rd.grid, lds, B.n, rd.rpw, A, V, B.r, U, r, rhs, part_slot(c, 0), part_slot(c, 1), NOGUARD, Deferred{})
+            if (which < 33) { if (B.cell_w == 8) UB_FRONT(8, 0, false); else UB_FRONT(16, 0, false); }
+            else if (which < 35) { if (B.cell_w == 8) UB_FRONT(8, FC_ALL, false); else UB_FRONT(16, FC_ALL, false); }
+            else { if (B.cell_w == 8) UB_FRONT(8, FC_ALL, true); else UB_FRONT(16, FC_ALL, true); }
 #undef UB_FRONT
         } break;
         case 32: LAUNCH(k_wsum, nblocks_for((size_t)B.nrow, TPB / 8), B.nrow, B.cs_w, (const double *)B.w_contrib, B.w_op, NOGUARD, InitArgs{}, 0, DS(0.0),
diff --git a/lorads_amd/csrc/hip/kernels.inc b/lorads_amd/csrc/hip/kernels.inc
--- a/lorads_amd/csrc/hip/kernels.inc
+++ b/lorads_amd/csrc/hip/kernels.inc
@@ -168,6 +168,23 @@
         if (live && threadIdx.x == 0) { ra.part_v[blockIdx.x] = vd[0]; ra.part_d[blockIdx.x] = vd[1]; }
     }
 }
+
+__device__ __forceinline__ double front_cw_m1(int wmode, int dual_on, double rho, double rho_dual, double cs0, double bb, double lam0,
+                                              double cvv, double wu) {
+    if (wmode == W_ADMM_V) {
+        const double cs = cs0 + (wu - cvv);
+        return ((cs - bb) - wu) * rho - lam0;
+    }
+    double lam = lam0;
+    if (dual_on) { const double l = lam0 + rho_dual * bb; lam = l + (-rho_dual) * cs0; }
+    return ((cs0 - bb) - cvv) * rho - lam;
+}
+struct WrecOut {
+    double2 *wrec;
+    const double *csum, *b, *lambda, *cv, *w_uv;
+    const int *row_idx;
+    DS rho;
+};
 
 template <int NS4, int NS>
 __global__ __launch_bounds__(TPB) void k_eval_cw_obj(int nrow, int ell_w, const int *__restrict__ a_p, const double *__restrict__ a_val,
@@ -690,7 +707,7 @@
 __device__ __forceinline__ double cg_wacc(double wa, double alpha, double wp) { return wa + alpha * wp; }
 __device__ __forceinline__ double cg0_alpha(double rr, double ww) { return rr / (rr + ww); }
 
-template <int LG, bool V2, int NS, int EW, bool CG0 = false>
+template <int LG, bool V2, int NS, int EW, bool CG0 = false, bool WR = false>
 __global__ __launch_bounds__(TPB) void k_spmm_ell(int n, int rpw, const int *__restrict__ adj_ptr, const int *__restrict__ adj_col,
                                                   const int *__restrict__ adj_con, const double *__restrict__ adj_a,
                                                   const int *__restrict__ ell_col, const int *__restrict__ ell_con,
@@ -698,7 +715,7 @@
                                                   const double *__restrict__ X, int r, int mode,
                                                   const double *xin, const double *__restrict__ rhs,
                                                   double *__restrict__ out, double *__restrict__ part, Guard g,
-                                                  Cg0Args u = Cg0Args{}) {
+                                                  Cg0Args u = Cg0Args{}, WrecOut wo = WrecOut{}) {
     __shared__ double sh[4];
     const Gate gt = gate_load(g);
     double rr = 0.0, ww = 0.0, wa0 = 0.0, wp0 = 0.0;
@@ -784,11 +801,31 @@
         }
     }
     if (CG0) {
+        double m_cs = 0.0, m_b = 0.0, m_lam = 0.0, m_cv = 0.0, m_rho = 0.0;
+        if constexpr (WR) {
+            if (gid < u.nw) {
+                const int gg = wo.row_idx ? wo.row_idx[gid] : gid;
+                m_cs = wo.csum[gg]; m_b = wo.b[gg]; m_lam = wo.lambda[gg]; m_cv = wo.cv[gid];
+            }
+            m_rho = dsv(wo.rho);
+        }
         const double alpha = cg0_alpha(rr, block_sum(ww, sh));
         const bool open = GATE_OPEN;
         const bool avg_only = !open && gt.vs != 0 && !(g.need && gt.vn == 0);
         if (open && blockIdx.x == 0 && threadIdx.x == 0 && u.shadow) *u.shadow = *u.st;
-        if (open && u.w_acc && gid < u.nw) {
+        if constexpr (WR) {
+            if (gid < u.nw) {
+                const double w_new = open ? cg_wacc(wa0, alpha, wp0) : wa0;
+                if (open) u.w_acc[gid] = w_new;
+                wo.wrec[gid] = make_double2(front_cw_m1(W_ADMM_V, 0, m_rho, 0.0, m_cs, m_b, m_lam, m_cv, w_new), w_new);
+                for (int i = gid + gridDim.x * TPB; i < u.nw; i += gridDim.x * TPB) {
+                    const int gg = wo.row_idx ? wo.row_idx[i] : i;
+                    const double w_i = open ? cg_wacc(u.w_acc[i], alpha, u.w_p[i]) : u.w_acc[i];
+                    if (open) u.w_acc[i] = w_i;
+                    wo.wrec[i] = make_double2(front_cw_m1(W_ADMM_V, 0, m_rho, 0.0, wo.csum[gg], wo.b[gg], wo.lambda[gg], wo.cv[i], w_i), w_i);
+                }
+            }
+        } else if (open && u.w_acc && gid < u.nw) {
             u.w_acc[gid] = cg_wacc(wa0, alpha, wp0);
             for (int i = gid + gridDim.x * TPB; i < u.nw; i += gridDim.x * TPB) u.w_acc[i] = cg_wacc(u.w_acc[i], alpha, u.w_p[i]);
         }
@@ -858,7 +895,11 @@
     const int *ell_col, *ell_con;
     const double *ell_a;
     const int *ell_dst, *sl_dst;
-    const double *csum, *b, *lambda, *cv, *w_uv;
+    union {
+        const double *csum;
+        const double2 *wrec;
+    };
+    const double *b, *lambda, *cv, *w_uv;
     const int *row_idx;
     DS rho, rho_dual;
     int dual_on;
@@ -868,20 +909,18 @@
     int nreset;
     int wt;
 };
+template <bool WR = false>
 __device__ __forceinline__ void front_cw_weights(const FrontCwArgs &A, double rho, double rho_dual, int i, double a, double &c1, double &c2) {
-    const int g = A.row_idx ? A.row_idx[i] : i;
-    const double cs0 = A.csum[g], bb = A.b[g], lam0 = A.lambda[g], cvv = A.cv[i], wu = A.w_uv[i];
-    double m1;
-    if (A.wmode == W_ADMM_V) {
-        const double cs = cs0 + (wu - cvv);
-        m1 = ((cs - bb) - wu) * rho - lam0;
+    if constexpr (WR) {
+        const double2 rec = A.wrec[i];
+        c1 = a * rec.x;
+        c2 = a * rec.y;
     } else {
-        double lam = lam0;
-        if (A.dual_on) { const double l = lam0 + rho_dual * bb; lam = l + (-rho_dual) * cs0; }
-        m1 = ((cs0 - bb) - cvv) * rho - lam;
-    }
-    c1 = a * m1;
-    c2 = a * wu;
+        const int g = A.row_idx ? A.row_idx[i] : i;
+        const double cs0 = A.csum[g], bb = A.b[g], lam0 = A.lambda[g], cvv = A.cv[i], wu = A.w_uv[i];
+        c1 = a * front_cw_m1(A.wmode, A.dual_on, rho, rho_dual, cs0, bb, lam0, cvv, wu);
+        c2 = a * wu;
+    }
 }
 struct EvalFinalArgs {
     const double *part_v, *part_d, *obj_part;
@@ -975,7 +1014,7 @@
         mine = l8 == u0 + u ? dsum : mine;
     }
 }
-template <int NS, int EW, int KC = 0, bool HO = false, int FC = 0>
+template <int NS, int EW, int KC = 0, bool HO = false, int FC = 0, bool WR = false>
 __global__ __launch_bounds__(TPB) void k_front_cw(int n, int rpw, std::conditional_t<HO, FrontCwHoArgs, FrontCwArgs> A,
                                                   const double *__restrict__ X, int r,
                                                   const double *__restrict__ xin, double *__restrict__ out,
@@ -1023,7 +1062,7 @@
     double k1[NH], k2[NH];
 #pragma unroll
     for (int h = 0; h < NH; ++h) {
-        front_cw_weights(A, rho, rho_dual, kc[h], ac[h], k1[h], k2[h]);
+        front_cw_weights<WR>(A, rho, rho_dual, kc[h], ac[h], k1[h], k2[h]);
         const bool mine = l8 + 8 * h < cnt;
         k1[h] = mine ? k1[h] : 0.0;
         k2[h] = mine ? k2[h] : 0.0;
@@ -1091,7 +1130,7 @@
     }
     for (int t = a0 + EW; t < a1; ++t) {
         double s1, s2, v[NS][W];
-        front_cw_weights(A, rho, rho_dual, A.sl_con[t], A.sl_a[t], s1, s2);
+        front_cw_weights<WR>(A, rho, rho_dual, A.sl_con[t], A.sl_a[t], s1, s2);
         if constexpr (RAW) SL::load_raw(X + (size_t)A.sl_col[t] * r, r, lane, v);
         else SL::load(X + (size_t)A.sl_col[t] * r, r, lane, v);
 #pragma unroll
diff --git a/lorads_amd/csrc/hip/lorads_hip.hip b/lorads_amd/csrc/hip/lorads_hip.hip
--- a/lorads_amd/csrc/hip/lorads_hip.hip
+++ b/lorads_amd/csrc/hip/lorads_hip.hip
@@ -347,6 +347,7 @@
     int cs_w = 0;
     int *cell_dst = nullptr, *cadj_dst = nullptr;
     double *w_contrib = nullptr;
+    double *wrec = nullptr;
     bool w0_ready = false;
     bool is_lp = false;
     int lp_nlev = 0;
@@ -692,6 +693,14 @@
     long long n_spec_enq = 0, n_spec_adopt = 0, n_spec_discard = 0, n_spec_blocked = 0;
     bool opt_handover_on_front = true;
     long long n_handover_front = 0, n_handover_alone = 0;
+    bool opt_front_wrec = true;
+    struct {
+        bool v_want = false;
+        bool v_ready = false;
+        double v_rho = 0.0;
+        long long v_at = 0;
+    } wrec;
+    long long n_wrec_v = 0, n_wrec_fly = 0;
     bool opt_exact_refresh = false, opt_split_front = false;
     bool final_pending = false;
     EvalFinalArgs final_args;
@@ -854,6 +863,7 @@
     if (getenv("LORADS_FRONT_CHAIN") && getenv("LORADS_FRONT_CHAIN")[0]) c->opt_front_chain = atoi(getenv("LORADS_FRONT_CHAIN")) & FC_ALL;
     c->opt_spec_front = env_on("LORADS_SPEC_FRONT");
     c->opt_handover_on_front = env_on("LORADS_HANDOVER_ON_FRONT");
+    c->opt_front_wrec = env_on("LORADS_FRONT_WREC");
     if (getenv("LORADS_SPEC_WINDOW")) c->spec_window = std::max(1, std::min(8, atoi(getenv("LORADS_SPEC_WINDOW"))));
     c->opt_fold_avg = env_on("LORADS_FOLD_AVG");
     c->opt_tile_update = env_on("LORADS_TILE_UPDATE");
@@ -1771,6 +1781,12 @@
     return 0;
 }
 
+int lorads_hip_front_wrec_stats(lorads_hip_ctx *c, int64_t out[2]) {
+    if (!c || !out) return fail_msg("front_wrec_stats: bad argument");
+    out[0] = c->n_wrec_v; out[1] = c->n_wrec_fly;
+    return 0;
+}
+
 int lorads_hip_row_deal_stats(lorads_hip_ctx *c, int32_t k, int out[3]) {
     if (!c || !out) return fail_msg("row_deal_stats: bad argument");
     if (k < 0 || k >= c->nb) return fail_msg("bad block");
diff --git a/lorads_amd/csrc/hip/sweep.inc b/lorads_amd/csrc/hip/sweep.inc
--- a/lorads_amd/csrc/hip/sweep.inc
+++ b/lorads_amd/csrc/hip/sweep.inc
@@ -86,12 +86,21 @@
     return row_deal(n, c->row_deal_cus);
 }
 int spmm_cw(lorads_hip_ctx *c, const Block &B, const double *w, const double *X, int mode, const double *xin, const double *rhs,
-            double *out, double *part, Guard g, const Cg0Args *cg0 = nullptr) {
+            double *out, double *part, Guard g, const Cg0Args *cg0 = nullptr, const WrecOut *wrec = nullptr) {
     const Shape sh = shape_for(B.r);
     const int grid = nblocks_for((size_t)B.n, TPB / sh.lg);
     const RowDeal rd = sh.lg == 8 ? row_deal_of(c, B) : RowDeal{TPB / sh.lg, grid};
     if (cg0) {
         if (!B.cell_w || !sh.v2 || mode != OP_CG) { c->launch_err = "CG iteration 0 in the operator: no kernel form for this cone"; return 0; }
+        if (wrec) {
+#define CG0W(NSV, EWV) LAUNCH((k_spmm_ell<8, true, NSV, EWV, true, true>), rd.grid, B.n, rd.rpw, B.cadj_ptr, B.cadj_col, B.cadj_con, B.cadj_a, \
+                              B.cell_col, B.cell_con, B.cell_a, w, X, B.r, mode, xin, rhs, (double *)nullptr, part, g, *cg0, *wrec)
+            if (sh.ns > 3 || sh.lg != 8) { c->launch_err = "weight record behind CG iteration 0: no kernel form for this cone"; return 0; }
+            if (B.cell_w == 8) { if (sh.ns == 1) CG0W(1, 8); else if (sh.ns == 2) CG0W(2, 8); else CG0W(3, 8); }
+            else { if (sh.ns == 1) CG0W(1, 16); else if (sh.ns == 2) CG0W(2, 16); else CG0W(3, 16); }
+#undef CG0W
+            return rd.grid;
+        }
         if (B.cell_w == 8) {
             NS_SWITCH(8, true, sh.ns, LAUNCH((k_spmm_ell<LG_, V2_, NS_, 8, true>), rd.grid, B.n, rd.rpw, B.cadj_ptr, B.cadj_col, B.cadj_con, B.cadj_a,
                                              B.cell_col, B.cell_con, B.cell_a, w, X, B.r, mode, xin, rhs, (double *)nullptr, part, g, *cg0))
@@ -307,7 +316,7 @@
 }
 
 int apply_operator(lorads_hip_ctx *c, Block &B, const double *V, const double *x, int mode, const double *rhs, double *out,
-                   double *part, Guard g, double *part_ww = nullptr, const Cg0Args *cg0 = nullptr) {
+                   double *part, Guard g, double *part_ww = nullptr, const Cg0Args *cg0 = nullptr, const WrecOut *wrec = nullptr) {
     const bool samp = c->prof && c->prof_target == 0 && c->prof_every < (1 << 20) && (c->n_matvec % c->prof_every == 0) &&
                       c->ev_next + 3 <= c->ev_pool.size();
     hipEvent_t e0 = nullptr, e1 = nullptr, e2 = nullptr;
@@ -336,7 +345,7 @@
             B.t_uv_valid = is_uv;
         }
         B.w0_ready = false;
-        grid = spmm_cw(c, B, w, V, mode, x, rhs, out, part, g, cg0);
+        grid = spmm_cw(c, B, w, V, mode, x, rhs, out, part, g, cg0, wrec);
     } else {
         const bool is_uv = (x == c->U + B.off && V == c->V + B.off) || (x == c->V + B.off && V == c->U + B.off);
         if (!(is_uv && B.t_uv_valid)) {
@@ -429,8 +438,16 @@
     A.wt = c->opt_wt_stores;
     return A;
 }
-int launch_front_cw(lorads_hip_ctx *c, const Solve &s, const FrontCwArgs &A, Guard g, Deferred d, const HandoverArgs *ho = nullptr) {
+bool front_wrec_form(const lorads_hip_ctx *c, const Block &B) {
+    return c->opt_front_wrec && B.wrec && c->opt_front_lds && (B.r + 15) / 16 <= 3 && (c->opt_front_chain & FC_ALL) == FC_ALL;
+}
+int launch_front_cw(lorads_hip_ctx *c, const Solve &s, const FrontCwArgs &A0, Guard g, Deferred d, const HandoverArgs *ho = nullptr,
+                    bool wr = false) {
     Block &B = *s.B;
+    FrontCwArgs A = A0;
+    wr = wr && front_wrec_form(c, B);
+    if (wr) A.wrec = (const double2 *)B.wrec;
+    ++(wr ? c->n_wrec_v : c->n_wrec_fly);
     double *r = c->cr + B.off, *rhs = c->rhs + B.off;
     double *pA = part_slot(c, 18), *pB = part_slot(c, 1);
     const RowDeal rd = row_deal_of(c, B);
@@ -450,7 +467,11 @@
     default: { constexpr int FC_ = 3; __VA_ARGS__; } break;        \
     } } while (0)
 #define FCW(EWV, HO, AV) NS_SWITCH(8, true, ns, LAUNCH((k_front_cw<NS_, EWV, 0, HO>), grid + lead, B.n, rd.rpw, AV, s.V, B.r, (const double *)s.x, r, rhs, pA, pB, g, d))
-#define FCWL(NSV, EWV, HO, AV) FC_SWITCH(LAUNCH_LDS((k_front_cw<NSV, EWV, 4, HO, FC_>), grid + lead, sizeof(double2) * 32 * 4 * NSV * 8, B.n, rd.rpw, AV, s.V, B.r, (const double *)s.x, r, rhs, pA, pB, g, d))
+#define FCWL(NSV, EWV, HO, AV)                                                                                                                   \
+    do {                                                                                                                                         \
+        if (wr) LAUNCH_LDS((k_front_cw<NSV, EWV, 4, HO, FC_ALL, true>), grid + lead, sizeof(double2) * 32 * 4 * NSV * 8, B.n, rd.rpw, AV, s.V, B.r, (const double *)s.x, r, rhs, pA, pB, g, d); \
+        else FC_SWITCH(LAUNCH_LDS((k_front_cw<NSV, EWV, 4, HO, FC_>), grid + lead, sizeof(double2) * 32 * 4 * NSV * 8, B.n, rd.rpw, AV, s.V, B.r, (const double *)s.x, r, rhs, pA, pB, g, d)); \
+    } while (0)
 #define FRONT(HO, AV)                                                                                                    \
     if (c->opt_front_lds && ns <= 3) {                                                                                   \
         if (B.cell_w == 8) { if (ns == 1) FCWL(1, 8, HO, AV); else if (ns == 2) FCWL(2, 8, HO, AV); else FCWL(3, 8, HO, AV); }     \
@@ -495,7 +516,10 @@
             A.dual_on = 1;
         }
         const Deferred d = c->pend.take_check_behind(s.front);
-        front_cw_started(c, s, launch_front_cw(c, s, A, s.front, d), tol);
+        const bool wr = c->wrec.v_ready && c->wrec.v_at == c->n_launch && ((s.st - c->st) & 1) && A.wmode == W_ADMM_V && !A.dual_on &&
+                        !c->pend.dual_owed() && memcmp(&rho, &c->wrec.v_rho, sizeof(double)) == 0 && B.t_uv_valid;
+        c->wrec.v_ready = false;
+        front_cw_started(c, s, launch_front_cw(c, s, A, s.front, d, nullptr, wr), tol);
         return;
     }
     if (fused_front(c, B)) {
@@ -567,7 +591,16 @@
         u.w_acc = rec ? B.w_uv : (double *)nullptr; u.w_p = B.w_op; u.nw = nw; u.shadow = shadow_of(c, s.st);
         u.avg_other = avg_other; u.avg_out = avg_out;
     }
-    const int npq = apply_operator(c, B, s.V, p, OP_CG, nullptr, Q, fuse0 ? pC : pA, g, pW, fuse0 ? &u : (const Cg0Args *)nullptr);
+    WrecOut wo{};
+    const bool vrec = fuse0 && c->wrec.v_want && rec && !B.diag_only && nw == B.nrow && front_wrec_form(c, B);
+    if (vrec) {
+        wo.wrec = (double2 *)B.wrec; wo.csum = c->csum; wo.b = c->b; wo.lambda = c->lambda; wo.cv = B.cv; wo.w_uv = B.w_uv;
+        wo.row_idx = B.row_idx_identity ? nullptr : B.row_idx; wo.rho = ds_rho(c, c->wrec.v_rho);
+    }
+    const int npq = apply_operator(c, B, s.V, p, OP_CG, nullptr, Q, fuse0 ? pC : pA, g, pW, fuse0 ? &u : (const Cg0Args *)nullptr,
+                                   vrec ? &wo : (const WrecOut *)nullptr);
+    c->wrec.v_ready = vrec;
+    c->wrec.v_at = c->n_launch;
     int nrr = npq;
     if (!fuse0) {
         if (v2_avg)
@@ -808,7 +841,12 @@
             solve_front(c, s, rho, tol, fresh0 ? c->st + 1 : nullptr, fresh0 ? 2 * c->nb - 1 : 0);
             const bool fold = eval_follows && stg == 2 * c->nb - 1 && c->nb == 1 && B.use_cw && c->opt_lazy_scalars &&
                               c->opt_fold_avg && B.nrow > 0 && nblocks_for((size_t)B.nrow, TPB / 64) <= c->maxpart;
+            c->wrec.v_ready = false;
+            c->wrec.v_want = eval_follows && c->nb == 1 && stg == 0 && c->opt_lazy_scalars && std::min(B.spec[half], maxit) == 1 &&
+                             front_cw_ok(c, B) && front_wrec_form(c, B) && !c->par_mode;
+            c->wrec.v_rho = rho;
             solve_iters(c, s, 0, std::min(B.spec[half], maxit), tol, maxit, fold);
+            c->wrec.v_want = false;
         }
         if (eval_follows && stg == 2 * c->nb - 1) {
             if (B.use_cw) {
diff --git a/lorads_amd/host.py b/lorads_amd/host.py
--- a/lorads_amd/host.py
+++ b/lorads_amd/host.py
@@ -720,6 +720,13 @@
         _check(lib.lorads_hip_handover_stats(ctx, out), "handover_stats")
         return dict(zip(["on_front", "alone"], [int(out[i]) for i in range(2)]))
 
+    def hip_front_wrec_stats(self):
+        lib, ctx = self._hip()
+        out = (C.c_int64 * 2)()
+        lib.lorads_hip_front_wrec_stats.argtypes = [C.c_void_p, C.POINTER(C.c_int64)]
+        _check(lib.lorads_hip_front_wrec_stats(ctx, out), "front_wrec_stats")
+        return dict(zip(["v_record", "on_the_fly"], [int(out[i]) for i in range(2)]))
+
     def hip_row_deal_stats(self, blk=0):
         lib, ctx = self._hip()
         out = (C.c_int * 3)()
```

After: 10430 (median of 6 runs). Within noise of the previous version (+0.9%).
